# facebookarchive/Surround360

Hardware: AMD Instinct MI355X
Metric: stereo-equirect frames/sec at 8K, 17-cam rig (higher is better)
Workload: dtype f32

## Files before the change

surround360_amd/csrc/api.hip:

```cpp
#include <algorithm>
#include <cstdio>
#include <cstdlib>
#include <cstring>
#include <fstream>
#include <mutex>
#include <sstream>

#include "../../include/s360.h"
#include "../../include/s360_debug.h"
#include "ctx.hpp"
#include "isp.hpp"
#include "render.hpp"

using namespace s360;

static thread_local std::string g_err;

namespace {
std::mutex g_ctxMu;
std::vector<unsigned long long> g_ctxLive;
unsigned long long g_ctxNext = 0;
}
namespace s360 {
bool context_alive(unsigned long long uid) {
// ... 428 lines not shown
    c->op_d.ensure(B * sizeof(void*));
    h2d(c, c->op_a.p, src, B * ns * 4);
    uchar4* down = c->op_b.as<uchar4>();
    float* gray = c->op_c.as<float>();
    float* alpha = gray + B * nd;
    std::vector<const uchar4*> tab(B);
    if (generic) {
      launch_resize_cubic_u8c4_generic(c->st, c->op_a.as<uchar4>(), sw, sh, ns, down, dw, dh, nd, batch);
      launch_gray_alpha(c->st, down, nd, nd, gray, alpha, nd, batch);
    } else {
      for (size_t b = 0; b < B; ++b) tab[b] = c->op_a.as<uchar4>() + ns * b;
      h2d(c, c->op_d.p, tab.data(), B * sizeof(void*));
      S360_HIP(hipMemsetAsync(down, 0x5a, B * nd * 4, c->st));
      launch_entry_downscale(c->st, nullptr, sw, sh, 0, down_out ? down : nullptr, down + B * nd, dw, dh, nd, batch,
                             c->op_d.as<const uchar4*>(), gray, alpha, nd);
    }
    if (down_out) d2h(c, down_out, down, B * nd * 4);
    d2h(c, gray_out, gray, B * nd * sizeof(float));
    d2h(c, alpha_out, alpha, B * nd * sizeof(float));
    if (tiled) *tiled = resize_cubic_u8c4_tiled_fits(sw, sh, dw, dh) ? 1 : 0;
  });
}

int s360_spherical_warp_map(s360_ctx* c, float* map_out, int dw, int dh, const s360_camera* cam, float l, float r,
                            float t, float b) {
  return guard(c, [&] {
    need(c && map_out && cam && dw > 0 && dh > 0, "bad argument");
    c->op_a.ensure((size_t)dw * dh * sizeof(float2));
    build_spherical_map(c, c->op_a.as<float2>(), dw, dh, *cam, l, r, t, b);
    d2h(c, map_out, c->op_a.p, (size_t)dw * dh * sizeof(float2));
  });
}
int s360_bicubic_remap_to_spherical(s360_ctx* c, uint8_t* dst, int dw, int dh, int dc, const uint8_t* src, int sw,
                                    int sh, int sc, const s360_camera* cam, float l, float r, float t, float b) {
  return guard(c, [&] {
    need(c && dst && src && cam, "null argument");
    need((dc == 3 || dc == 4) && (sc == 3 || sc == 4), "channels must be 3 or 4");
    need(!(sc == 4 && dc == 3), "4-channel source: the reference's remap() re-creates the destination with the source's type (ImageWarper.cpp:173) - pass a 4-channel destination");
    FrameState& F = frame_state(c);
    const size_t sn = (size_t)sw * sh, dn = (size_t)dw * dh;
    c->op_a.ensure(dn * sizeof(float2));
    c->op_b.ensure(sn * 4);
    c->op_c.ensure(sn * sizeof(uchar4));
    c->op_d.ensure(dn * sizeof(uchar4));
    build_spherical_map(c, c->op_a.as<float2>(), dw, dh, *cam, l, r, t, b);
    h2d(c, c->op_b.p, src, sn * sc);
    launch_bgr_to_bgra(c->st, c->op_b.as<uint8_t>(), sc, c->op_c.as<uchar4>(), sn);
    launch_remap_cubic_u8c4(c->st, c->op_c.as<uchar4>(), sw, sh, c->op_a.as<float2>(), c->op_d.as<uchar4>(), dw, dh,
                            F.tab.dev, 0, 0, 1);
    if (dc == 4) {
      d2h(c, dst, c->op_d.p, dn * 4);
    } else {
      c->op_e.ensure(dn * 3);
      launch_pack_bgr(c->st, c->op_d.as<uchar4>(), dw, dh, c->op_e.as<uint8_t>());
      d2h(c, dst, c->op_e.p, dn * 3);
    }
  });
}
int s360_combine_lazy_novel_views(s360_ctx* c, const uint8_t* image_l, const uint8_t* image_r, const float* flow_l_to_r,
                                  const float* flow_r_to_l, uint8_t* chunk_l, uint8_t* chunk_r) {
  return guard(c, [&] {
    need(c && image_l && image_r && flow_l_to_r && flow_r_to_l && chunk_l && chunk_r, "null argument");
    FrameState& F = frame_state(c);
    const s360_geometry& g = c->g;
    const int P = F.P, ow = g.overlap_image_width, camH = g.cam_image_height, stripW = c->P.eqr_width / P;
    const size_t on = (size_t)ow * camH, sn = (size_t)stripW * camH;
    c->op_a.ensure(2 * on * 4);
    c->op_b.ensure(2 * on * sizeof(float2));
    c->op_c.ensure(2 * sn * 4);
    h2d(c, c->op_a.p, image_l, on * 4);
    h2d(c, c->op_a.as<uint8_t>() + on * 4, image_r, on * 4);
    h2d(c, c->op_b.p, flow_l_to_r, on * sizeof(float2));
    h2d(c, c->op_b.as<float2>() + on, flow_r_to_l, on * sizeof(float2));
    NovelViewParams nv;
    nv.overlapW = ow; nv.camH = camH; nv.stripW = stripW; nv.numNovelViews = g.num_novel_views;
    nv.numPairs = 1; nv.numLocal = 1;
    nv.camImageWidthHalf = float(g.cam_image_width) * 0.5f;
    nv.disp = g.verge_at_infinity_slab_displacement;
    launch_novel_view(c->st, c->op_a.as<uchar4>(), c->op_b.as<float2>(), c->op_c.as<uchar4>(), nv, 0, 1, F.tab.dev);
    d2h(c, chunk_l, c->op_c.p, sn * 4);
    d2h(c, chunk_r, c->op_c.as<uint8_t>() + sn * 4, sn * 4);
  });
}
static void morph_views_resident(s360_ctx* c, int w, int h, const double* shifts, int n, uint8_t* out_merged, uint8_t* out_from_l,
                                 uint8_t* out_from_r) {
  FrameState& F = frame_state(c);
  const size_t px = (size_t)w * h, V = n;
  c->op_c.ensure(V * px * 4 * (1 + (out_from_l ? 1 : 0) + (out_from_r ? 1 : 0)));
  c->op_d.ensure(V * sizeof(double));
  h2d(c, c->op_d.p, shifts, V * sizeof(double));
  uchar4* merged = c->op_c.as<uchar4>();
  uchar4* fromL = out_from_l ? merged + V * px : nullptr;
  uchar4* fromR = out_from_r ? merged + V * px * (out_from_l ? 2 : 1) : nullptr;
  const char* e = std::getenv("S360_MORPH_VPB");
  {
    ProfScope ps(c->prof, "morph_views");
    launch_morph_views(c->st, c->op_a.as<uchar4>(), c->op_a.as<uchar4>() + px, c->op_b.as<float2>(), c->op_b.as<float2>() + px, w, h,
                       c->op_d.as<double>(), n, merged, fromL, fromR, F.tab.dev, e ? std::atoi(e) : 0);
  }
  d2h(c, out_merged, merged, V * px * 4);
  if (fromL) d2h(c, out_from_l, fromL, V * px * 4);
  if (fromR) d2h(c, out_from_r, fromR, V * px * 4);
}
int s360_generate_novel_views(s360_ctx* c, const uint8_t* image_l, const uint8_t* image_r, const float* flow_l_to_r,
                              const float* flow_r_to_l, int w, int h, const double* shifts, int n, uint8_t* out_merged,
                              uint8_t* out_from_l, uint8_t* out_from_r) {
  return guard(c, [&] {
    need(c && image_l && image_r && flow_l_to_r && flow_r_to_l && shifts && out_merged, "null argument");
    need(w > 0 && h > 0, "image size must be positive");
    need(n >= 1, "at least one shift is required");
    const size_t px = (size_t)w * h;
    c->op_a.ensure(2 * px * 4);
    c->op_b.ensure(2 * px * sizeof(float2));
    h2d(c, c->op_a.p, image_l, px * 4);
    h2d(c, c->op_a.as<uint8_t>() + px * 4, image_r, px * 4);
    h2d(c, c->op_b.p, flow_l_to_r, px * sizeof(float2));
    h2d(c, c->op_b.as<float2>() + px, flow_r_to_l, px * sizeof(float2));
    morph_views_resident(c, w, h, shifts, n, out_merged, out_from_l, out_from_r);
  });
}
int s360_interpolate_views(s360_ctx* c, const char* alg, const uint8_t* image_l, const uint8_t* image_r, int w, int h,
                           const double* shifts, int n, uint8_t* out_merged, uint8_t* out_from_l, uint8_t* out_from_r,
                           float* out_flow_l_to_r, float* out_flow_r_to_l) {
  return guard(c, [&] {
    need(c && alg && image_l && image_r && shifts && out_merged, "null argument");
    need(w >= 4 && h >= 4, "image too small: the reference's bilinear taps need a 2x2 image after the x0.5 entry downscale (PixFlow.h:457-475)");
    need(n >= 1, "at least one shift is required");
    const PixFlowConsts pc = pixflow_consts_by_name(alg);
    const size_t px = (size_t)w * h;
    c->op_a.ensure(2 * px * 4);
    c->op_b.ensure(2 * px * sizeof(float2));
    h2d(c, c->op_a.p, image_l, px * 4);
    h2d(c, c->op_a.as<uint8_t>() + px * 4, image_r, px * 4);
    for (int d = 0; d < 2; ++d) {
      FlowBatch fb;
      fb.add_images(c->op_a.as<uchar4>(), 2, px);
      fb.add_flow(d, 1 - d, c->op_b.as<float2>() + px * d);
      c->flow->compute(c->st, pc, fb, w, h, d == 0 ? S360_HINT_LEFT : S360_HINT_RIGHT);
    }
    morph_views_resident(c, w, h, shifts, n, out_merged, out_from_l, out_from_r);
    if (out_flow_l_to_r) d2h(c, out_flow_l_to_r, c->op_b.p, px * sizeof(float2));
    if (out_flow_r_to_l) d2h(c, out_flow_r_to_l, c->op_b.as<float2>() + px, px * sizeof(float2));
  });
}
int s360_flatten_layers_deghost_prefer_base(s360_ctx* c, const uint8_t* bottom_layer, const uint8_t* top_layer, int w,
                                            int h, uint8_t* out) {
  return guard(c, [&] {
    need(c && bottom_layer && top_layer && out && w > 0 && h > 0, "bad argument");
    FrameState& F = frame_state(c);
    const size_t n = (size_t)w * h;
    c->op_a.ensure(n * 4); c->op_b.ensure(n * 4); c->op_c.ensure(n * 4);
    h2d(c, c->op_a.p, bottom_layer, n * 4);
    h2d(c, c->op_b.p, top_layer, n * 4);
    launch_flatten(c->st, c->op_a.as<uchar4>(), c->op_b.as<uchar4>(), c->op_c.as<uchar4>(), w, h, 0, F.tab.dev);
    d2h(c, out, c->op_c.p, n * 4);
  });
}
int s360_offset_horizontal_wrap(s360_ctx* c, const uint8_t* src, int w, int h, int channels, float offset,
                                uint8_t* out) {
  return guard(c, [&] {
    need(c && src && out && w > 0 && h > 0, "bad argument");
    need(channels == 3 || channels == 4, "channels must be 3 or 4");
    const size_t n = (size_t)w * h;
    c->op_a.ensure(n * 4); c->op_b.ensure(n * 4);
    if (channels == 4) {
      h2d(c, c->op_a.p, src, n * 4);
    } else {
      c->op_c.ensure(n * 3);
      h2d(c, c->op_c.p, src, n * 3);
      launch_bgr_to_bgra(c->st, c->op_c.as<uint8_t>(), 3, c->op_a.as<uchar4>(), n);
    }
    launch_assemble_pano(c->st, c->op_a.as<uchar4>(), 1, h, w, offset, c->op_b.as<uchar4>(), w, h);
    if (channels == 4) {
      d2h(c, out, c->op_b.p, n * 4);
    } else {
      launch_pack_bgr(c->st, c->op_b.as<uchar4>(), w, h, c->op_c.as<uint8_t>());
      d2h(c, out, c->op_c.p, n * 3);
    }
  });
}
int s360_feather_alpha_channel(s360_ctx* c, const uint8_t* src, int w, int h, int erode_size, uint8_t* out) {
  return guard(c, [&] {
    need(c && src && out && w > 0 && h > 0, "bad argument");
    need(erode_size >= 1 && erode_size <= 32, "erode_size must be in 1..32");
    need(erode_size % 2 == 1, "erode_size must be odd (it is the GaussianBlur kernel size, CvUtil.cpp:151)");
    const size_t n = (size_t)w * h;
    c->op_a.ensure(n * 4); c->op_b.ensure(n * 4);
    h2d(c, c->op_a.p, src, n * 4);
    if (erode_size == c->P.std_alpha_feather_size) {
      dev_feather_alpha_to_ext(c, c->op_a.as<uchar4>(), w, h, c->op_b.as<uchar4>(), w);
    } else {
      const std::vector<int> taps = feather_gauss_taps(erode_size);
      c->op_e.ensure(taps.size() * sizeof(int));
      h2d(c, c->op_e.p, taps.data(), taps.size() * sizeof(int));
      dev_feather_alpha_to_ext(c, c->op_a.as<uchar4>(), w, h, c->op_b.as<uchar4>(), w, erode_size, c->op_e.as<int>());
    }
    d2h(c, out, c->op_b.p, n * 4);
  });
}
int s360_pole_to_side_flow(s360_ctx* c, const uint8_t* side, const uint8_t* pole, int pole_rows, uint8_t* warped_out,
                           float* flow_out) {
  return guard(c, [&] {
    need(c && side && pole && warped_out && pole_rows > 0, "bad argument");
    need(c->bottom_idx >= 0, "rig has no bottom camera (pole ramp uses its fov, TRSP:461)");
    const int W = c->P.eqr_width, H = c->P.eqr_height;
    need(pole_rows <= H, "pole_rows larger than eqr_height");
    const int extW = int(float(W) * 1.2f);
    const size_t en = (size_t)W * H, pn = (size_t)W * pole_rows, xn = (size_t)extW * pole_rows;
    c->op_a.ensure(en * 4); c->op_b.ensure(pn * 4); c->op_c.ensure(2 * xn * 4); c->op_d.ensure(xn * sizeof(float2));
    c->op_e.ensure(en * 4);
    h2d(c, c->op_a.p, side, en * 4);
    h2d(c, c->op_b.p, pole, pn * 4);
    uchar4* ext = c->op_c.as<uchar4>();
    dev_feather_alpha_to_ext(c, c->op_a.as<uchar4>(), W, pole_rows, ext, extW);
    launch_extend_wrap(c->st, c->op_b.as<uchar4>(), nullptr, W, pole_rows, ext + xn, extW);
    (void)flow_engine(c, 1);
    FlowBatch fb;
    fb.add_images(ext, 2, xn);
    fb.add_flow(0, 1, c->op_d.as<float2>());
    c->flow_pole->compute(c->st, pixflow_consts_by_name(c->P.polar_flow_alg), fb, extW, pole_rows, S360_HINT_DOWN);
    dev_pole_unit_post(c, ext + xn, c->op_d.as<float2>(), W, pole_rows, extW, c->op_e.as<uchar4>(), H);
    d2h(c, warped_out, c->op_e.p, en * 4);
    if (flow_out) d2h(c, flow_out, c->op_d.p, xn * sizeof(float2));
  });
}
int s360_sharpen(s360_ctx* c, uint8_t* bgr, int w, int h, float sharpening) {
  return guard(c, [&] {
    need(c && bgr && w > 1 && h > 1, "bad argument");
    const size_t n = (size_t)w * h;
    c->op_a.ensure(n * 3); c->op_b.ensure(n * 4); c->op_c.ensure(n * 4); c->op_d.ensure(sharpen_scratch_bytes(w, h));
    h2d(c, c->op_a.p, bgr, n * 3);
    launch_bgr_to_bgra(c->st, c->op_a.as<uint8_t>(), 3, c->op_b.as<uchar4>(), n);
    launch_sharpen(c->st, c->op_b.as<uchar4>(), c->op_c.as<uchar4>(), c->op_d.as<float>(), w, h, 1.0f + sharpening);
    launch_pack_bgr(c->st, c->op_b.as<uchar4>(), w, h, c->op_a.as<uint8_t>());
    d2h(c, bgr, c->op_a.p, n * 3);
  });
}

int s360_frame_upload_side(s360_ctx* c, int side_idx, const uint8_t* img, int w, int h, int channels) {
  return frame_guard(c, [&] { need(c && img && w > 0 && h > 0, "bad argument"); frame_upload_side(c, side_idx, img, w, h, channels); });
}
int s360_frame_upload_top(s360_ctx* c, const uint8_t* bgr, int w, int h) {
  return frame_guard(c, [&] { need(c && bgr && w > 0 && h > 0, "bad argument"); frame_upload_pole(c, true, bgr, w, h); });
}
int s360_frame_upload_bottom(s360_ctx* c, const uint8_t* bgr, int w, int h) {
  return frame_guard(c, [&] { need(c && bgr && w > 0 && h > 0, "bad argument"); frame_upload_pole(c, false, bgr, w, h); });
}
int s360_frame_upload_raw(s360_ctx* c, s360_isp* isp, int camera, const uint16_t* raw16, int w, int h) {
  return frame_guard(c, [&] { need(c && isp && raw16 && w > 0 && h > 0, "bad argument"); frame_upload_raw(c, isp, camera, raw16, 16, w, h); });
}
int s360_frame_upload_packed(s360_ctx* c, s360_isp* isp, int camera, const uint8_t* frame, int bits, int w, int h) {
  return frame_guard(c, [&] {
    need(c && isp && frame && w > 0 && h > 0, "bad argument");
    need(bits == 8 || bits == 12, "packed frames are 8 or 12 bits per pixel");
    frame_upload_raw(c, isp, camera, frame, bits, w, h);
  });
}
int s360_frame_upload_pole_removal(s360_ctx* c, const uint8_t* bottom2, const uint8_t* mask, const uint8_t* mask2, int w,
                                   int h) {
  return frame_guard(c, [&] {
    need(c && bottom2 && mask && mask2 && w > 0 && h > 0, "bad argument");
    frame_upload_pole_removal(c, bottom2, mask, mask2, w, h);
  });
}
int s360_frame_set_prev_pole_removal(s360_ctx* c, const float* flow, const uint8_t* bottom_image, const uint8_t* bottom_image2,
                                     int w, int h) {
  return frame_guard(c, [&] {
    need(c && flow && bottom_image && bottom_image2 && w > 0 && h > 0, "bad argument");
    FrameState& F = frame_state(c);
    const size_t n = (size_t)w * h;
    const int prv = F.last_pr;
    F.prImgs[prv].ensure(2 * n * sizeof(uchar4));
    F.prFlow[prv].ensure(n * sizeof(float2));
    h2d(c, F.prImgs[prv].as<uchar4>(), bottom_image, n * sizeof(uchar4));
    h2d(c, F.prImgs[prv].as<uchar4>() + n, bottom_image2, n * sizeof(uchar4));
    h2d(c, F.prFlow[prv].p, flow, n * sizeof(float2));
    S360_HIP(hipStreamSynchronize(c->st));
    F.have_prev_pr = true;
    F.prevPrGot = 0;
  });
}
int s360_frame_render_pairs(s360_ctx* c, int p0, int p1, int use_prev) {
  return frame_guard(c, [&] { need(c, "null ctx"); frame_render_pairs(c, p0, p1, use_prev); });
}
int s360_frame_finish(s360_ctx* c, int pole_mask, int use_prev) {
  return frame_guard(c, [&] { need(c, "null ctx"); frame_finish(c, pole_mask, use_prev); });
}
int s360_frame_render(s360_ctx* c, int use_prev) {
  return frame_guard(c, [&] {
    need(c, "null ctx");
    frame_render_pairs(c, 0, (int)c->rig.side.size(), use_prev);
    frame_finish(c, 15, use_prev);
  });
}
int s360_set_frame_slots(s360_ctx* c, int n) {
  return frame_guard(c, [&] { need(c, "null ctx"); set_frame_slots(c, n); });
}
int s360_select_frame_slot(s360_ctx* c, int k) {
  return frame_guard(c, [&] {
    need(c, "null ctx");
    need(k >= 0 && k < (int)std::max<size_t>(c->slots.size(), 1), "frame slot out of range");
    c->slot = k;
  });
}
int s360_frame_render_batch(s360_ctx* c, int use_prev) {
  return frame_guard(c, [&] { need(c, "null ctx"); frame_render_batch(c, use_prev); });
}
// ... 295 lines not shown
    png_fetch(c, lk, plan, c->op_d, c->op_b, nullptr, nullptr, nullptr, out, cap, n_out, false);
  });
}
void* s360_host_alloc(size_t bytes) {
  void* p = nullptr;
  if (bytes == 0 || hipHostMalloc(&p, bytes, hipHostMallocPortable) != hipSuccess) {
    (void)hipGetLastError();
    g_err = "s360_host_alloc: hipHostMalloc failed";
    return nullptr;
  }
  std::lock_guard<std::mutex> lk(g_pinMu);
  g_pinBlocks.emplace_back(static_cast<const char*>(p), bytes);
  return p;
}
void s360_host_free(void* p) {
  if (!p) return;
  {
    std::lock_guard<std::mutex> lk(g_pinMu);
    for (size_t i = 0; i < g_pinBlocks.size(); ++i)
      if (g_pinBlocks[i].first == p) { g_pinBlocks.erase(g_pinBlocks.begin() + i); break; }
  }
  (void)hipHostFree(p);
}
int s360_frame_uploads_complete(s360_ctx* c) {
  if (!c) return S360_ERR_INVALID_ARG;
  return guard_l(c, [&](std::unique_lock<std::recursive_mutex>& lk) {
    if (!c->haveUploaded) return;
    if (!c->evUpHost) S360_HIP(hipEventCreateWithFlags(&c->evUpHost, hipEventDisableTiming | hipEventBlockingSync));
    S360_HIP(hipEventRecord(c->evUpHost, c->stUp));
    const hipEvent_t ev = c->evUpHost;
    lk.unlock();
    const hipError_t rc = hipEventSynchronize(ev);
    lk.lock();
    S360_HIP(rc);
  });
}

int s360_set_cubemap_output(s360_ctx* c, int face_w, int face_h, const char* format) {
  return frame_guard(c, [&] {
    need(c, "null ctx");
    if (face_w == 0 || face_h == 0) { c->cube_fw = c->cube_fh = 0; return; }
    need(format, "bad argument");
    const std::string f(format);
    if (f != "video" && f != "photo")
      throw Error(S360_ERR_INVALID_ARG, "unexpected cubemap format: " + f + ". valid formats are: video,photo");
    need(face_w > 0 && face_h > 0 && face_w <= 16384 && face_h <= 16384, "cubemap face size must be in 1..16384 (0 = off)");
    (void)cube_maps(c, face_w, face_h, f == "video");
    c->cube_fw = face_w; c->cube_fh = face_h; c->cube_video = f == "video";
  });
}
int s360_frame_cubemap_size(s360_ctx* c, int whc[3]) {
  return guard(c, [&] {
    need(c && whc, "bad argument");
    if (c->cube_fw <= 0 || c->cube_fh <= 0) throw Error(S360_ERR_STATE, "the cubemap output is off (s360_set_cubemap_output)");
    whc[0] = c->cube_video ? 3 * c->cube_fw : c->cube_fw;
    whc[1] = c->cube_video ? 4 * c->cube_fh : 12 * c->cube_fh;
    whc[2] = 3;
  });
}
static void ensure_download_stream(s360_ctx* c) {
  if (!c->stDown) S360_HIP(hipStreamCreateWithFlags(&c->stDown, hipStreamNonBlocking));
  if (!c->evDown) S360_HIP(hipEventCreateWithFlags(&c->evDown, hipEventDisableTiming | hipEventBlockingSync));
  if (!c->downErr) {
    S360_HIP(hipHostMalloc((void**)&c->downErr, 4 * sizeof(unsigned), hipHostMallocDefault));
    std::memset(c->downErr, 0, 4 * sizeof(unsigned));
  }
}
static int cube_buffer(s360_ctx* c, FrameState& F, int age) {
  need(F.frames_done > age, "that frame has not been rendered");
  need(age == 0 || ((c->pipeline || c->two_outputs) && F.outBGR[F.out_cur ^ 1].p),
       "age 1 needs two output buffers (s360_set_frame_pipelining or s360_set_output_double_buffer)");
  const int b = age == 0 ? F.out_cur : F.out_cur ^ 1;
  if (F.cubeFrame[b] != F.frames_done - 1 - age || !F.cubeBGR[b].p)
    throw Error(S360_ERR_STATE, "that frame was rendered without s360_set_cubemap_output");
  return b;
}
static int download_cubemap_impl(s360_ctx* c, int slot, int age, uint8_t* out_bgr) {
  if (!c) return S360_ERR_INVALID_ARG;
  return guard_l(c, [&](std::unique_lock<std::recursive_mutex>& lk) {
    need(out_bgr && (age == 0 || age == 1), "bad argument (age is 0 = latest enqueued frame or 1 = the one before)");
    FrameState& F = slot_state(c, slot);
    const int b = cube_buffer(c, F, age);
    ensure_download_stream(c);
    if (!F.downRead[b]) S360_HIP(hipEventCreateWithFlags(&F.downRead[b], hipEventDisableTiming));
    S360_HIP(hipStreamWaitEvent(c->stDown, F.outDone[b], 0));
    S360_HIP(hipMemcpyAsync(out_bgr, F.cubeBGR[b].p, (size_t)F.cubeOutW[b] * F.cubeOutH[b] * 3, hipMemcpyDeviceToHost, c->stDown));
    if (F.outErrDev[b].p) S360_HIP(hipMemcpyAsync(c->downErr, F.outErrDev[b].p, 3 * sizeof(unsigned), hipMemcpyDeviceToHost, c->stDown));
    S360_HIP(hipEventRecord(F.downRead[b], c->stDown));
    S360_HIP(hipEventRecord(c->evDown, c->stDown));
    const hipEvent_t ev = c->evDown;
    const unsigned* errw = F.outErrDev[b].p ? c->downErr : nullptr;
    lk.unlock();
    const hipError_t rc = hipEventSynchronize(ev);
    lk.lock();
    S360_HIP(rc);
    if (errw && (errw[0] | errw[1] | errw[2])) {
      for (FlowEngine* e : {c->flow.get(), c->flow_pole.get(), c->flow_pr.get()})
        if (e) (void)e->take_error(c->st);
      throw Error(S360_ERR_HIP, "banded sweep timed out waiting for a neighbour band (results invalid)");
    }
  });
}
int s360_frame_download_cubemap(s360_ctx* c, int age, uint8_t* out_bgr) { return download_cubemap_impl(c, -1, age, out_bgr); }
int s360_frame_download_cubemap_slot(s360_ctx* c, int slot, int age, uint8_t* out_bgr) {
  if (slot < 0) return S360_ERR_INVALID_ARG;
  return download_cubemap_impl(c, slot, age, out_bgr);
}
size_t s360_frame_cubemap_png_bound(s360_ctx* c) {
  size_t n = 0;
  if (!c) return 0;
  (void)guard(c, [&] {
    if (c->cube_fw > 0 && c->cube_fh > 0)
      n = PngPlan::make(c->cube_video ? 3 * c->cube_fw : c->cube_fw, c->cube_video ? 4 * c->cube_fh : 12 * c->cube_fh).file_bound;
  });
  return n;
}
static int download_cubemap_png_impl(s360_ctx* c, int slot, int age, uint8_t* out, size_t cap, size_t* n_out) {
  if (!c) return S360_ERR_INVALID_ARG;
  return guard_l(c, [&](std::unique_lock<std::recursive_mutex>& lk) {
    need(out && n_out && (age == 0 || age == 1), "bad argument (age is 0 = latest enqueued frame or 1 = the one before)");
    FrameState& F = slot_state(c, slot);
    const int b = cube_buffer(c, F, age);
    if (F.cubePngFrame[b] != F.frames_done - 1 - age || !F.cubePngFile[b].p)
      throw Error(S360_ERR_STATE, "that frame was rendered without s360_set_png_encode");
    if (!F.downRead[b]) S360_HIP(hipEventCreateWithFlags(&F.downRead[b], hipEventDisableTiming));
    png_fetch(c, lk, F.cubePngPlan[b], F.cubePngMeta[b], F.cubePngFile[b], F.outDone[b], F.downRead[b], F.outErrDev[b].p, out, cap, n_out);
  });
}
int s360_frame_download_cubemap_png(s360_ctx* c, int age, uint8_t* out, size_t cap, size_t* n_out) {
  return download_cubemap_png_impl(c, -1, age, out, cap, n_out);
}
int s360_frame_download_cubemap_png_slot(s360_ctx* c, int slot, int age, uint8_t* out, size_t cap, size_t* n_out) {
  if (slot < 0) return S360_ERR_INVALID_ARG;
  return download_cubemap_png_impl(c, slot, age, out, cap, n_out);
}

int s360_frame_cubemap(s360_ctx* c, int face_w, int face_h, const char* format, int whc[3], uint8_t* out_bgr) {
  return frame_guard(c, [&] {
    need(c && format && whc, "bad argument");
    const std::string f(format);
    if (f != "video" && f != "photo")
      throw Error(S360_ERR_INVALID_ARG, "unexpected cubemap format: " + f + ". valid formats are: video,photo");
    need(face_w > 0 && face_h > 0 && face_w <= 16384 && face_h <= 16384, "cubemap face size must be in 1..16384");
    whc[0] = f == "video" ? 3 * face_w : face_w;
    whc[1] = f == "video" ? 4 * face_h : 12 * face_h;
    whc[2] = 3;
    if (!out_bgr) return;
    int ow = 0, oh = 0;
    wait_finish_stream(c);
    frame_cubemap(c, face_w, face_h, f == "video", &ow, &oh);
    d2h(c, out_bgr, frame_state(c).cubeOut.p, (size_t)ow * oh * 3);
  });
}
static const void* frame_u8_source(s360_ctx* c, FrameState& F, const std::string& n, int idx, bool pack_eye, int& w, int& h, int& ch) {
  const s360_geometry& g = c->g;
  const int W = c->P.eqr_width, H = c->P.eqr_height, P = F.P;
  const void* src = nullptr;
  w = 0; h = 0; ch = 4;
  const int nloc = F.side_p1 - F.side_p0;
  if (n == "projection") {
    need(idx >= 0 && idx < P && F.sc->proj.p, "projection not available");
    w = g.cam_image_width; h = g.cam_image_height;
    src = F.sc->proj.as<uchar4>() + (size_t)w * h * idx;
  } else if (n == "overlap_l" || n == "overlap_r") {
    need(idx >= F.side_p0 && idx < F.side_p1 && F.overlaps[F.last_side].p, "overlap not available");
    w = g.overlap_image_width; h = g.cam_image_height;
    const int j = idx - F.side_p0 + (n == "overlap_r" ? nloc : 0);
    src = F.overlaps[F.last_side].as<uchar4>() + (size_t)w * h * j;
  } else if (n == "side_pano_l" || n == "side_pano_r") {
    const int e = n == "side_pano_r";
    need(F.panoDbg[e].p, "enable keep_intermediates before rendering");
    w = W; h = H; src = F.panoDbg[e].p;
  } else if (n == "top_spherical") {
    need(F.sc->topSph.p, "not available"); w = W; h = g.top_rows; src = F.sc->topSph.p;
  } else if (n == "bottom_spherical") {
    need(F.sc->botSph.p, "not available"); w = W; h = g.bottom_rows; src = F.sc->botSph.p;
  } else if (n == "pole_warped") {
    need(idx >= 0 && idx < 4 && F.sc->poleWarped[idx].p, "not available"); w = W; h = H; src = F.sc->poleWarped[idx].p;
  } else if (n == "extended_side" || n == "extended_fisheye") {
    need(idx >= 0 && idx < 4 && F.extImgs[F.last_pole].p, "not available");
    w = F.extW; h = idx < 2 ? F.poleRowsT : F.poleRowsB;
    const int slot = n == "extended_side" ? idx : (idx < 2 ? 4 : 5);
    src = F.extImgs[F.last_pole].as<uchar4>() + F.extStride * slot;
  } else if (n == "bottom_image" || n == "bottom_image2") {
    need(F.prImgs[F.last_pr].p && F.have_prev_pr, "not available (pole removal not run)");
    w = F.poleW; h = F.poleH;
    src = F.prImgs[F.last_pr].as<uchar4>() + (n == "bottom_image2" ? (size_t)w * h : 0);
  } else if (n == "eye_l" || n == "eye_r") {
    const int e = n == "eye_r";
    need(F.pano[e].p, "not available");
    w = W; h = H; ch = 3;
    if (pack_eye) {
      c->op_f.ensure((size_t)w * h * 3);
      wait_finish_stream(c);
      launch_pack_bgr(c->st, F.pano[e].as<uchar4>(), w, h, c->op_f.as<uint8_t>());
      src = c->op_f.p;
    }
  } else {
    throw Error(S360_ERR_INVALID_ARG, "unknown intermediate name: " + n);
  }
  return src;
}
int s360_frame_get_u8(s360_ctx* c, const char* name, int idx, int whc[3], uint8_t* dst) {
  return frame_guard(c, [&] {
    need(c && name && whc, "bad argument");
    int w = 0, h = 0, ch = 4;
    const void* src = frame_u8_source(c, frame_state(c), name, idx, dst != nullptr, w, h, ch);
    whc[0] = w; whc[1] = h; whc[2] = ch;
    if (dst) d2h(c, dst, src, (size_t)w * h * ch);
  });
}
size_t s360_png_bound_c(int w, int h, int channels) {
  size_t n = 0;
  (void)guard(nullptr, [&] { n = PngPlan::make(w, h, channels).file_bound; });
  return n;
}
int s360_encode_png_c(s360_ctx* c, const uint8_t* px, int w, int h, int channels, uint8_t* out, size_t cap, size_t* n_out) {
  if (!c) return S360_ERR_INVALID_ARG;
  return guard_l(c, [&](std::unique_lock<std::recursive_mutex>& lk) {
    need(px && out && n_out && w > 0 && h > 0, "bad argument");
    const PngPlan plan = PngPlan::make(w, h, channels);
    const size_t nb = (size_t)w * h * channels;
    c->op_a.ensure((nb + 3) & ~(size_t)3);
    c->op_b.ensure(plan.file_bound);
    S360_HIP(hipMemcpyAsync(c->op_a.p, px, nb, hipMemcpyHostToDevice, c->st));
    png_encode_enqueue(c->st, c->op_a.as<uint8_t>(), plan, c->op_c, c->op_d, c->op_b.as<uint8_t>());
    S360_HIP(hipStreamSynchronize(c->st));
    png_fetch(c, lk, plan, c->op_d, c->op_b, nullptr, nullptr, nullptr, out, cap, n_out, false);
  }, false);
}
static void png_batch_prepare(s360_ctx* c, s360_ctx::PngBatch& B, const std::vector<PngPlan>& plans) {
  if (!B.events) {
    S360_HIP(hipEventCreateWithFlags(&B.evEnc, hipEventDisableTiming));
    S360_HIP(hipEventCreateWithFlags(&B.evRead, hipEventDisableTiming));
    S360_HIP(hipEventCreateWithFlags(&B.evAfter, hipEventDisableTiming));
    B.events = true;
  }
  if (B.haveEnc && hipEventQuery(B.evEnc) != hipSuccess) {
    (void)hipGetLastError();
    S360_HIP(hipEventSynchronize(B.evEnc));
  }
  B.haveEnc = false;
  B.plan = PngBatchPlan::make(plans);
  auto grow = [](void*& p, size_t& have, size_t want) {
    if (have >= want) return;
    if (p) (void)hipHostFree(p);
    p = nullptr;
    have = 0;
    S360_HIP(hipHostMalloc(&p, want, hipHostMallocDefault));
    have = want;
  };
  grow(B.tabHost, B.tabHostBytes, PngBatchPlan::table_bytes(plans.size(), (size_t)B.plan.nbands));
  grow(B.metaHost, B.metaHostBytes, B.plan.meta_records * sizeof(PngBandMeta));
}
static void png_batch_run(s360_ctx* c, s360_ctx::PngBatch& B, const uint8_t* const* px) {
  if (B.haveRead) S360_HIP(hipStreamWaitEvent(c->st, B.evRead, 0));
  png_batch_enqueue(c->st, px, B.plan, B.table, B.tabHost, B.scratch, B.meta, B.files);
  S360_HIP(hipMemcpyAsync(B.metaHost, B.meta.p, B.plan.meta_records * sizeof(PngBandMeta), hipMemcpyDeviceToHost, c->st));
  S360_HIP(hipEventRecord(B.evEnc, c->st));
  B.haveEnc = true;
  ++B.gen;
}
static void png_batch_fetch(s360_ctx* c, std::unique_lock<std::recursive_mutex>& lk, s360_ctx::PngBatch& B, int i, uint8_t* out, size_t cap,
                            size_t* n_out, bool release) {
  if (!B.haveEnc) throw Error(S360_ERR_STATE, "no PNG batch has been encoded");
  need(i >= 0 && (size_t)i < B.plan.img.size(), "PNG index out of range");
  need(out && n_out, "bad argument");
  const PngPlan plan = B.plan.img[(size_t)i];
  const uint8_t* file = B.files.as<uint8_t>() + B.plan.file_off[(size_t)i];
  const PngBandMeta* mh = static_cast<const PngBandMeta*>(B.metaHost) + B.plan.meta0[(size_t)i];
  const unsigned long long gen = B.gen;
  const char* too_small = "png: output buffer too small (s360_frame_state_png_bound / s360_png_bound_c give the size to allocate)";
  if (!c->stDown) S360_HIP(hipStreamCreateWithFlags(&c->stDown, hipStreamNonBlocking));
  std::vector<PngBandMeta> m((size_t)plan.nbands + 1);
  const bool known = hipEventQuery(B.evEnc) == hipSuccess;
  if (!known) (void)hipGetLastError();
  size_t nbytes = std::min(cap, plan.file_bound);
  if (known) {
    std::memcpy(m.data(), mh, m.size() * sizeof(PngBandMeta));
    nbytes = (size_t)m[(size_t)plan.nbands].file_off;
    if (nbytes > plan.file_bound || nbytes + 28 > cap) throw Error(S360_ERR_INVALID_ARG, too_small);
  }
  hipEvent_t ev = nullptr;
  S360_HIP(hipEventCreateWithFlags(&ev, hipEventDisableTiming | hipEventBlockingSync));
  struct Drop { hipEvent_t e; ~Drop() { (void)hipEventDestroy(e); } } drop{ev};
  S360_HIP(hipStreamWaitEvent(c->stDown, B.evEnc, 0));
  S360_HIP(hipMemcpyAsync(out, file, nbytes, hipMemcpyDeviceToHost, c->stDown));
  S360_HIP(hipEventRecord(B.evRead, c->stDown));
  B.haveRead = true;
  S360_HIP(hipEventRecord(ev, c->stDown));
  if (release) lk.unlock();
  const hipError_t rc = hipEventSynchronize(ev);
  if (release) lk.lock();
  S360_HIP(rc);
  if (B.gen != gen) throw Error(S360_ERR_STATE, "the PNG batch was replaced by a later encode while this file was being fetched");
  if (!known) {
    std::memcpy(m.data(), mh, m.size() * sizeof(PngBandMeta));
    const size_t end = (size_t)m[(size_t)plan.nbands].file_off;
    if (end > plan.file_bound || end + 28 > cap) throw Error(S360_ERR_INVALID_ARG, too_small);
  }
  if (release) lk.unlock();
  const size_t n = png_finish_host(out, cap, plan, m.data(), png_crc_threads());
  if (release) lk.lock();
  *n_out = n;
}
int s360_encode_png_batch(s360_ctx* c, int n, const uint8_t* const* px, const int* w, const int* h, const int* channels, uint8_t* const* out,
                          const size_t* cap, size_t* n_out) {
  if (!c) return S360_ERR_INVALID_ARG;
  return guard_l(c, [&](std::unique_lock<std::recursive_mutex>& lk) {
    need(n > 0 && n <= 4096 && px && w && h && channels && out && cap && n_out, "bad argument");
    std::vector<PngPlan> plans;
    std::vector<size_t> at;
    size_t total = 0;
    for (int i = 0; i < n; ++i) {
      need(px[i] && out[i], "bad argument");
      plans.push_back(PngPlan::make(w[i], h[i], channels[i]));
      at.push_back(total);
      total += ((size_t)w[i] * h[i] * channels[i] + 15) & ~(size_t)15;
    }
    c->op_a.ensure(total);
    std::vector<const uint8_t*> dev;
    for (int i = 0; i < n; ++i) {
      dev.push_back(c->op_a.as<uint8_t>() + at[(size_t)i]);
      S360_HIP(hipMemcpyAsync(c->op_a.as<uint8_t>() + at[(size_t)i], px[i], (size_t)w[i] * h[i] * channels[i], hipMemcpyHostToDevice, c->st));
    }
    png_batch_prepare(c, c->opPng, plans);
    png_batch_run(c, c->opPng, dev.data());
    S360_HIP(hipStreamSynchronize(c->st));
    for (int i = 0; i < n; ++i) png_batch_fetch(c, lk, c->opPng, i, out[i], cap[i], &n_out[i], false);
  }, false);
}
int s360_frame_encode_state_pngs(s360_ctx* c, int n, const char* const* names, const int* idx) {
  return frame_guard(c, [&] {
    need(c && n > 0 && n <= 4096 && names && idx, "bad argument");
    FrameState& F = frame_state(c);
    std::vector<PngPlan> plans;
    std::vector<const uint8_t*> px;
    for (int i = 0; i < n; ++i) {
      need(names[i] != nullptr, "bad argument");
      int w = 0, h = 0, ch = 0;
      const void* src = frame_u8_source(c, F, names[i], idx[i], false, w, h, ch);
      need(ch == 4 && src, "only the 4-channel intermediates are encoded as state images");
      plans.push_back(PngPlan::make(w, h, 4));
      px.push_back(static_cast<const uint8_t*>(src));
    }
    s360_ctx::PngBatch& B = c->statePng;
    png_batch_prepare(c, B, plans);
    if (c->st2) {
      S360_HIP(hipEventRecord(B.evAfter, c->st2));
      S360_HIP(hipStreamWaitEvent(c->st, B.evAfter, 0));
    }
    png_batch_run(c, B, px.data());
  });
}
size_t s360_frame_state_png_bound(s360_ctx* c, int i) {
  size_t n = 0;
  if (!c) return 0;
  (void)guard(c, [&] {
    const s360_ctx::PngBatch& B = c->statePng;
    if (!B.haveEnc) throw Error(S360_ERR_STATE, "no PNG batch has been encoded");
    need(i >= 0 && (size_t)i < B.plan.img.size(), "PNG index out of range");
    n = B.plan.img[(size_t)i].file_bound;
  });
  return n;
}
int s360_frame_download_state_png(s360_ctx* c, int i, uint8_t* out, size_t cap, size_t* n_out) {
  if (!c) return S360_ERR_INVALID_ARG;
  return guard_l(c, [&](std::unique_lock<std::recursive_mutex>& lk) { png_batch_fetch(c, lk, c->statePng, i, out, cap, n_out, true); });
}
static const char* const kNotDecodable = "not a banded PNG file of this decoder";
int s360_png_decodable(const uint8_t* file, size_t n, int whc[3], int* band_rows) {
  return guard(nullptr, [&] {
    need(whc && band_rows, "bad argument");
    PngBandedInfo I;
    if (!png_parse_banded(file, n, I)) throw Error(S360_ERR_INVALID_ARG, kNotDecodable);
    whc[0] = I.w; whc[1] = I.h; whc[2] = I.channels;
    *band_rows = I.band_rows;
  });
}
[[noreturn]] static void png_fail(s360_ctx* c, int image, int reason, const std::string& msg) {
  c->pngDecFailImage = image;
  c->pngDecFailReason = reason;
  throw Error(S360_ERR_INVALID_ARG, msg);
}
static std::vector<PngBandedInfo> png_parse_all(s360_ctx* c, int n, const uint8_t* const* files, const size_t* bytes) {
  c->pngDecFailImage = -1;
  c->pngDecFailReason = S360_PNG_DECODE_FAILURE_NONE;
  std::vector<PngBandedInfo> info((size_t)n);
  for (int i = 0; i < n; ++i) {
    need(files[i] != nullptr, "bad argument");
    if (!png_parse_banded(files[i], bytes[i], info[(size_t)i]))
      png_fail(c, i, S360_PNG_DECODE_FAILURE_NOT_DECODABLE, "png decode: image " + std::to_string(i) + ": " + kNotDecodable);
  }
  return info;
}
static void png_decode_checked(s360_ctx* c, int n, const uint8_t* const* files, const std::vector<PngBandedInfo>& info, const std::vector<uint8_t*>& dst) {
  try {
    png_decode_run(c->st, c->pngDec, std::vector<const uint8_t*>(files, files + n), info, dst, c->pngDecStats, &c->prof);
  } catch (const PngDecodeError& e) {
    c->pngDecFailImage = e.image;
    c->pngDecFailReason = S360_PNG_DECODE_FAILURE_DAMAGED;
    throw;
  }
}
int s360_png_decode_failure(s360_ctx* c, int* image, int* reason) {
  if (!c) return S360_ERR_INVALID_ARG;
  return guard(c, [&] {
    need(image && reason, "bad argument");
    *image = c->pngDecFailImage;
    *reason = c->pngDecFailReason;
  });
}
int s360_decode_png_batch(s360_ctx* c, int n, const uint8_t* const* files, const size_t* bytes, uint8_t* const* out, const size_t* cap,
                          int* whc_out) {
  if (!c) return S360_ERR_INVALID_ARG;
  return guard_l(c, [&](std::unique_lock<std::recursive_mutex>&) {
    need(n > 0 && n <= 4096 && files && bytes && out && cap, "bad argument");
    const std::vector<PngBandedInfo> info = png_parse_all(c, n, files, bytes);
    std::vector<size_t> at;
    size_t total = 0;
    for (int i = 0; i < n; ++i) {
      const PngBandedInfo& I = info[(size_t)i];
      const size_t nb = (size_t)I.w * I.h * I.channels;
      need(out[i] != nullptr, "bad argument");
      if (cap[i] < nb) png_fail(c, i, S360_PNG_DECODE_FAILURE_MISMATCH, "png decode: image " + std::to_string(i) + ": output buffer too small");
      at.push_back(total);
      total += (nb + 15) & ~(size_t)15;
    }
    c->op_a.ensure(total);
    std::vector<uint8_t*> dst;
    for (int i = 0; i < n; ++i) dst.push_back(c->op_a.as<uint8_t>() + at[(size_t)i]);
    png_decode_checked(c, n, files, info, dst);
    for (int i = 0; i < n; ++i) {
      const PngBandedInfo& I = info[(size_t)i];
      S360_HIP(hipMemcpyAsync(out[i], dst[(size_t)i], (size_t)I.w * I.h * I.channels, hipMemcpyDeviceToHost, c->st));
      if (whc_out) { whc_out[3 * i] = I.w; whc_out[3 * i + 1] = I.h; whc_out[3 * i + 2] = I.channels; }
    }
    S360_HIP(hipStreamSynchronize(c->st));
  }, false);
}
int s360_png_decode_stats(s360_ctx* c, uint64_t out[4]) {
  if (!c) return S360_ERR_INVALID_ARG;
  return guard(c, [&] {
    need(out != nullptr, "bad argument");
    for (int k = 0; k < 4; ++k) out[k] = c->pngDecStats[k];
  });
}
int s360_png_decode_round_histogram(s360_ctx* c, uint64_t hist[66]) {
  if (!c) return S360_ERR_INVALID_ARG;
  return guard(c, [&] {
    need(hist != nullptr, "bad argument");
    for (int k = 0; k < 66; ++k) hist[k] = c->pngDecStats[4 + k];
  });
}
static void prev_side_arrived(FrameState& F, int pair, unsigned bits) {
  if (F.prevSideGot.size() < (size_t)F.P) F.prevSideGot.resize((size_t)F.P, 0);
  unsigned char& g = F.prevSideGot[(size_t)pair];
  g |= (unsigned char)bits;
  if (g == 15) { g = 0; F.have_prev_side = true; }
}
static void prev_pole_arrived(s360_ctx* c, FrameState& F, int unit, unsigned bits) {
  unsigned char& g = F.prevPoleGot[unit];
  g |= (unsigned char)bits;
  if (g == 7) {
    g = 0;
    F.extW = int(float(c->P.eqr_width) * 1.2f);
    F.extStride = (size_t)F.extW * std::max(c->g.top_rows, c->g.bottom_rows);
    F.poleRowsT = c->g.top_rows;
    F.poleRowsB = c->g.bottom_rows;
    F.have_prev_pole = true;
  }
}
static void prev_pr_arrived(FrameState& F, unsigned bits) {
  F.prevPrGot |= (unsigned char)bits;
  if (F.prevPrGot == 7) { F.prevPrGot = 0; F.have_prev_pr = true; }
}
static void prev_side_block(FrameState& F, int pair, int& j, int& n) {
  need(pair >= 0 && pair < F.P, "pair_idx out of range");
  if (!F.partition_declared) { F.side_p0 = 0; F.side_p1 = F.P; }
  need(pair >= F.side_p0 && pair < F.side_p1, "pair_idx outside the block declared with s360_frame_set_partition");
  j = pair - F.side_p0;
  n = F.side_p1 - F.side_p0;
}
int s360_frame_set_prev_images_png(s360_ctx* c, int n, const char* const* names, const int* idx, const uint8_t* const* files,
                                   const size_t* bytes) {
  return frame_guard(c, [&] {
    need(c && n > 0 && n <= 4096 && names && idx && files && bytes, "bad argument");
    FrameState& F = frame_state(c);
    const std::vector<PngBandedInfo> info = png_parse_all(c, n, files, bytes);
    const size_t on = (size_t)c->g.overlap_image_width * c->g.cam_image_height;
    const int extW = int(float(c->P.eqr_width) * 1.2f);
    const size_t xs = (size_t)extW * std::max(c->g.top_rows, c->g.bottom_rows);
    struct Arrival { int kind, k; unsigned bits; };
    std::vector<uint8_t*> dst;
    std::vector<Arrival> arr;
    int prW = 0, prH = 0;
    for (int i = 0; i < n; ++i) {
      need(names[i] != nullptr, "bad argument");
      const std::string nm(names[i]);
      const PngBandedInfo& I = info[(size_t)i];
      int w = 0, h = 0;
      uchar4* p = nullptr;
      if (nm == "overlap_l" || nm == "overlap_r") {
// ... 252 lines not shown
```

surround360_amd/csrc/render.hip:

```cpp
#include "render.hpp"

#include "isp.hpp"

#include <algorithm>
#include <cmath>
#include <cstdlib>
#include <cstring>

#include "devmath.hpp"

namespace s360 {

std::vector<int> feather_gauss_taps(int erode_size) {
  const int n = erode_size;
  std::vector<int> ik(std::max(n, 1));
  std::vector<float> k(std::max(n, 1));
  const double sigma = erode_size / 2.0f;
  const double sigmaX = sigma > 0 ? sigma : ((n - 1) * 0.5 - 1) * 0.3 + 0.8;
  const double scale2X = -0.5 / (sigmaX * sigmaX);
  double sum = 0;
  for (int i = 0; i < n; ++i) {
    const double x = i - (n - 1) * 0.5;
    k[i] = (float)std::exp(scale2X * x * x);
    sum += k[i];
// ... 441 lines not shown
  s360_ctx::PackedMap& pk = *cache.e.back();
  pk.packed.ensure((size_t)batch * dw * dh * sizeof(unsigned));
  pk.tiles.ensure((size_t)batch * remap_packed_tiles(dw, dh) * 16);
  launch_remap_pack_map(st, map, sw, sh, dw, dh, pk.packed.as<unsigned>(), pk.tiles.p, batch);
  S360_HIP(hipEventCreateWithFlags(&pk.ready, hipEventDisableTiming));
  S360_HIP(hipEventRecord(pk.ready, st));
  pk.sw = sw;
  pk.sh = sh;
  return pk;
}

static void side_stage(s360_ctx* c, const std::vector<int>& slotIds, int p0, int p1, int use_prev) {
  const s360_geometry& g = c->g;
  const int P = (int)c->rig.side.size();
  if (p0 < 0 || p1 > P || p1 < p0) throw Error(S360_ERR_INVALID_ARG, "bad pair range");
  if (c->P.eqr_width % P != 0)
    throw Error(S360_ERR_INVALID_ARG, "eqr_width must be evenly divisible by the number of cameras");
  if (g.num_novel_views != c->P.eqr_width / P)
    throw Error(S360_ERR_INVALID_ARG, "numNovelViews != eqr_width / numCams for this rig");
  Profiler& prof = c->prof;
  hipStream_t st = c->st;
  const int camW = g.cam_image_width, camH = g.cam_image_height, ow = g.overlap_image_width;
  const int stripW = c->P.eqr_width / P;
  const size_t pn = (size_t)camW * camH, on = (size_t)ow * camH;
  const int n = p1 - p0;
  std::vector<FrameState*> Fs;
  for (int k : slotIds) {
    SlotScope ss(c, k);
    FrameState& F = frame_state(c);
    if (!F.have_side) throw Error(S360_ERR_STATE, "side images not uploaded");
    for (int p = p0; p < p1; ++p)
      if (!((F.side_uploaded >> p) & 1) || !((F.side_uploaded >> ((p + 1) % P)) & 1))
        throw Error(S360_ERR_STATE, "side image of camera " + std::to_string(((F.side_uploaded >> p) & 1) ? (p + 1) % P : p) +
                                        " not uploaded (needed by pair " + std::to_string(p) + ")");
    F.sc->proj.ensure(P * pn * sizeof(uchar4));
    F.strips.ensure((size_t)2 * P * camH * stripW * sizeof(uchar4));
    Fs.push_back(&F);
  }
  ensure_maps(c);
  if (n == 0) {
    if (c->evSideSrcFree) { S360_HIP(hipEventRecord(c->evSideSrcFree, st)); c->haveSideSrcFree = true; }
    if (c->pipeline && c->haveStripsFree) S360_HIP(hipStreamWaitEvent(st, c->evStripsFree, 0));
    if (c->pipeline) S360_HIP(hipEventRecord(c->evSideDone, st));
    return;
  }
  if (2 * n * (int)Fs.size() > kMaxFlows) throw Error(S360_ERR_INVALID_ARG, "too many flows for one batch");
  wait_for_uploads(c, st);
  bool usePrev = use_prev != 0;
  for (FrameState* F : Fs) usePrev = usePrev && F->have_prev_side && F->side_p0 == p0 && F->side_p1 == p1;
  for (FrameState* F : Fs) F->cur_side = usePrev ? F->last_side ^ 1 : F->last_side;
  for (FrameState* Fp : Fs) {
    FrameState& F = *Fp;
    const size_t sn = (size_t)F.srcW * F.srcH;
    {
      ProfScope ps(prof, "project_side");
      std::vector<char> need(P, 0);
      for (int p = p0; p < p1; ++p) need[p] = need[(p + 1) % P] = 1;
      for (int i = 0; i < P;) {
        if (!need[i]) { ++i; continue; }
        int j = i;
        while (j < P && need[j]) ++j;
        s360_ctx::PackedMap& pk = ensure_packed(c, c->sidePk, c->sideMaps.as<float2>(), F.srcW, F.srcH, camW, camH, P, st);
        launch_remap_cubic_u8c4_packed(st, F.sideSrc.as<uchar4>() + sn * i, F.srcW, F.srcH, c->sideMaps.as<float2>() + pn * i,
                                       pk.packed.as<unsigned>() + pn * i,
                                       (const char*)pk.tiles.p + 16 * remap_packed_tiles(camW, camH) * i,
                                       F.sc->proj.as<uchar4>() + pn * i, camW, camH, F.tab.dev, 0, 0, 1, j - i);
        i = j;
      }
    }
    const int cur = F.cur_side;
    F.overlaps[cur].ensure(2 * n * on * sizeof(uchar4));
    F.sideFlows.ensure(2 * n * on * sizeof(float2));
    {
      ProfScope ps(prof, "crop_overlaps");
      launch_crop_overlaps(st, F.sc->proj.as<uchar4>(), camW, camH, P, ow, F.overlaps[cur].as<uchar4>(), p0, p1);
    }
  }
  if (c->evSideSrcFree) {
    S360_HIP(hipEventRecord(c->evSideSrcFree, st));
    c->haveSideSrcFree = true;
  }
  {
    (void)flow_engine(c, 0);
    const PixFlowConsts pc = pixflow_consts_by_name(c->P.side_flow_alg);
    for (FrameState* F : Fs) F->have_prev_side = false;
    auto build = [&](bool ltor, bool rtol) {
      FlowBatch fb;
      for (size_t k = 0; k < Fs.size(); ++k) {
        FrameState& F = *Fs[k];
        const int cur = F.cur_side, prv = cur ^ 1;
        const int base = (int)fb.images.size();
        fb.add_images(F.overlaps[cur].as<uchar4>(), 2 * n, on);
        if (usePrev) fb.add_prev_images(F.overlaps[prv].as<uchar4>(), 2 * n, on);
        float2* out = F.sideFlows.as<float2>();
        const float2* pf = usePrev ? F.sideFlows.as<float2>() : nullptr;
        if (ltor)
          for (int j = 0; j < n; ++j) fb.add_flow(base + j, base + n + j, out + on * j, pf ? pf + on * j : nullptr);
        if (rtol)
          for (int j = 0; j < n; ++j) fb.add_flow(base + n + j, base + j, out + on * (n + j), pf ? pf + on * (n + j) : nullptr);
      }
      return fb;
    };
    if (pc.maxPercentage == 0) {
      c->flow->compute(st, pc, build(true, true), ow, camH, S360_HINT_LEFT);
    } else {
      c->flow->compute(st, pc, build(true, false), ow, camH, S360_HINT_LEFT);
      c->flow->compute(st, pc, build(false, true), ow, camH, S360_HINT_RIGHT);
    }
  }
  for (FrameState* Fp : Fs) {
    FrameState& F = *Fp;
    const int cur = F.cur_side;
    {
      ProfScope ps(prof, "novel_view");
      NovelViewParams nv;
      nv.overlapW = ow; nv.camH = camH; nv.stripW = stripW; nv.numNovelViews = g.num_novel_views;
      nv.numPairs = P; nv.numLocal = n;
      nv.camImageWidthHalf = float(camW) * 0.5f;
      nv.disp = g.verge_at_infinity_slab_displacement;
      if (c->pipeline && c->haveStripsFree) S360_HIP(hipStreamWaitEvent(st, c->evStripsFree, 0));
      launch_novel_view(st, F.overlaps[cur].as<uchar4>(), F.sideFlows.as<float2>(), F.strips.as<uchar4>(), nv, p0,
                        p1, F.tab.dev);
    }
    F.side_p0 = p0;
    F.side_p1 = p1;
    F.have_prev_side = true;
    F.last_side = cur;
    F.prevSideGot.clear();
  }
  if (c->pipeline) S360_HIP(hipEventRecord(c->evSideDone, st));
}
void frame_render_pairs(s360_ctx* c, int p0, int p1, int use_prev) { side_stage(c, {c->slot}, p0, p1, use_prev); }

void dev_feather_alpha_to_ext(s360_ctx* c, const uchar4* pano, int cols, int rows, uchar4* ext, int extW, int erode_size,
                              const int* taps) {
  FrameState& F = frame_state(c);
  hipStream_t st = c->st;
  const size_t n = (size_t)cols * rows;
  F.a8a.ensure(n);
  F.a8b.ensure(n);
  const int e = erode_size >= 0 ? erode_size : c->P.std_alpha_feather_size;
  const int ksize = erode_size >= 0 ? erode_size : F.tab.gauss_ksize;
  const int* gik = erode_size >= 0 ? taps : F.tab.gik.as<int>();
  launch_erode_alpha(st, pano, F.a8b.as<uint8_t>(), cols, rows, e);
  if (ksize > 1) {
    launch_gauss_u8(st, F.a8b.as<uint8_t>(), F.a8a.as<uint8_t>(), cols, rows, gik, ksize / 2);
    launch_extend_wrap(st, pano, F.a8a.as<uint8_t>(), cols, rows, ext, extW);
  } else {
    launch_extend_wrap(st, pano, F.a8b.as<uint8_t>(), cols, rows, ext, extW);
  }
}

void dev_pole_unit_post(s360_ctx* c, const uchar4* extFisheye, const float2* flow, int cols, int rows, int extW,
                        uchar4* warped_out, int eqrH) {
  FrameState& F = frame_state(c);
  PoleWarpParams pw;
  pw.cols = cols; pw.rows = rows; pw.extW = extW;
  pw.maxBlendX = int(float(cols) * (1.2f - 1.0f));
  pw.poleCameraRadius = c->ramp.poleCameraRadius;
  pw.phiRampStart = c->ramp.phiRampStart;
  pw.phiMid = c->ramp.phiMid;
  pw.phiRampEnd = c->ramp.phiRampEnd;
  F.sc->warpedExt.ensure((size_t)extW * rows * sizeof(uchar4));
  F.sc->warpPacked.ensure((size_t)extW * rows * sizeof(unsigned));
  F.sc->warpTiles.ensure(remap_packed_tiles(extW, rows) * 16);
  launch_pole_warp_packed(c->st, extFisheye, flow, F.sc->warpedExt.as<uchar4>(), pw, F.tab.dev, F.sc->warpPacked.as<unsigned>(),
                          F.sc->warpTiles.p);
  launch_pole_finish(c->st, F.sc->warpedExt.as<uchar4>(), warped_out, eqrH, pw);
}

namespace {
struct FinishStream {
  s360_ctx* c;
  hipStream_t saved, savedProf;
  explicit FinishStream(s360_ctx* c_) : c(c_), saved(c_->st), savedProf(c_->prof.st) {
    if (c->pipeline) {
      c->st = c->st2;
      c->prof.st = c->st2;
      S360_HIP(hipStreamWaitEvent(c->st2, c->evSideDone, 0));
    }
  }
  ~FinishStream() {
    c->st = saved;
    c->prof.st = savedProf;
  }
};
}

static void finish_stage(s360_ctx* c, const std::vector<int>& slotIds, int pole_mask, int use_prev, int phases = 3,
                         int composite_mask = -1) {
  if (composite_mask < 0) composite_mask = pole_mask;
  if (!(phases & 1)) pole_mask = 0;
  const s360_geometry& g = c->g;
  Profiler& prof = c->prof;
  FinishStream finishStream(c);
  hipStream_t st = c->st;
  const int P = (int)c->rig.side.size(), W = c->P.eqr_width, H = c->P.eqr_height, camH = g.cam_image_height, stripW = W / P;
  const size_t en = (size_t)W * H;
  if (!c->P.enable_top) { pole_mask &= ~3; composite_mask &= ~3; }
  if (!c->P.enable_bottom) { pole_mask &= ~12; composite_mask &= ~12; }
  const int rowsT = g.top_rows, rowsB = g.bottom_rows;
  const int extW = int(float(W) * 1.2f);
  const size_t xs = (size_t)extW * std::max(rowsT, rowsB);
  auto rowsOf = [&](int u) { return u < 2 ? rowsT : rowsB; };
  if (pole_mask) ensure_maps(c);
  bool usePrev = use_prev != 0 && pole_mask != 0;
  for (int k : slotIds) {
    SlotScope ss(c, k);
    FrameState& F = frame_state(c);
    usePrev = usePrev && F.have_prev_pole && F.extW == extW && F.poleRowsT == rowsT && F.poleRowsB == rowsB;
  }
  for (int k : slotIds) {
    SlotScope ss(c, k);
    FrameState& F = frame_state(c);
    F.cur_pole = usePrev ? F.last_pole ^ 1 : F.last_pole;
  }
  for (int k : slotIds) {
    SlotScope ss(c, k);
    FrameState& F = frame_state(c);
    if (!(phases & 1)) {
      if (!F.pano[0].p || !F.pano[1].p) throw Error(S360_ERR_STATE, "composite without assembled panoramas (s360_frame_pole_units first)");
      continue;
    }
    if (!F.strips.p) throw Error(S360_ERR_STATE, "no strips rendered for this frame");
    for (int e = 0; e < 2; ++e) F.pano[e].ensure(en * sizeof(uchar4));
    F.sc->panoTmp.ensure(en * sizeof(uchar4));
    {
      ProfScope ps(prof, "assemble_pano");
      const float sh = g.zero_parallax_novel_view_shift_pixels;
      launch_assemble_pano(st, F.strips.as<uchar4>(), P, camH, stripW, sh, F.pano[0].as<uchar4>(), W, H);
      launch_assemble_pano(st, F.strips.as<uchar4>() + (size_t)P * camH * stripW, P, camH, stripW, -sh,
                           F.pano[1].as<uchar4>(), W, H);
    }
    if (F.keep_intermediates)
      for (int e = 0; e < 2; ++e) {
        F.panoDbg[e].ensure(en * sizeof(uchar4));
        S360_HIP(hipMemcpyAsync(F.panoDbg[e].p, F.pano[e].p, en * sizeof(uchar4), hipMemcpyDeviceToDevice, st));
      }
    if (!pole_mask) continue;
    const int cur = F.cur_pole;
    F.extImgs[cur].ensure(6 * xs * sizeof(uchar4));
    F.poleFlows.ensure(4 * xs * sizeof(float2));
    uchar4* ext = F.extImgs[cur].as<uchar4>();
    wait_for_uploads(c, st);
    {
      ProfScope ps(prof, "project_pole");
      if (pole_mask & 3) {
        if (!F.have_top) throw Error(S360_ERR_STATE, "top image not uploaded");
        F.sc->topSph.ensure((size_t)W * rowsT * sizeof(uchar4));
        const int yfs = rowsT - 1 - c->P.std_alpha_feather_size;
        s360_ctx::PackedMap& pk = ensure_packed(c, c->topPk, c->topMap.as<float2>(), F.topW, F.topH, W, rowsT, 1, st);
        launch_remap_cubic_u8c4_packed(st, F.topSrc.as<uchar4>(), F.topW, F.topH, c->topMap.as<float2>(),
                                       pk.packed.as<unsigned>(), pk.tiles.p, F.sc->topSph.as<uchar4>(), W, rowsT,
                                       F.tab.dev, 1, yfs, c->P.std_alpha_feather_size);
        launch_extend_wrap(st, F.sc->topSph.as<uchar4>(), nullptr, W, rowsT, ext + 4 * xs, extW);
      }
      if (pole_mask & 12) {
        if (!F.have_bottom) throw Error(S360_ERR_STATE, "bottom image not uploaded");
        F.sc->botSph.ensure((size_t)W * rowsB * sizeof(uchar4));
        const int yfs = rowsB - 1 - c->P.std_alpha_feather_size;
        if (c->P.enable_pole_removal) {
          dev_pole_removal(c, F, use_prev != 0);
          s360_ctx::PackedMap& pk = ensure_packed(c, c->botPk, c->botMap.as<float2>(), F.poleW, F.poleH, W, rowsB, 1, st);
          launch_remap_cubic_u8c4_packed(st, F.prMerged.as<uchar4>(), F.poleW, F.poleH, c->botMap.as<float2>(),
                                         pk.packed.as<unsigned>(), pk.tiles.p, F.sc->botSph.as<uchar4>(), W, rowsB,
                                         F.tab.dev, 2, yfs, c->P.std_alpha_feather_size);
        } else {
          s360_ctx::PackedMap& pk = ensure_packed(c, c->botPk, c->botMap.as<float2>(), F.poleW, F.poleH, W, rowsB, 1, st);
          launch_remap_cubic_u8c4_packed(st, F.botSrc.as<uchar4>(), F.poleW, F.poleH, c->botMap.as<float2>(),
                                         pk.packed.as<unsigned>(), pk.tiles.p, F.sc->botSph.as<uchar4>(), W, rowsB,
                                         F.tab.dev, 1, yfs, c->P.std_alpha_feather_size);
        }
        launch_extend_wrap(st, F.sc->botSph.as<uchar4>(), nullptr, W, rowsB, ext + 5 * xs, extW);
      }
    }
    {
      ProfScope ps(prof, "pole_prepare");
      if (pole_mask & 12) {
        for (int e = 0; e < 2; ++e) {
          F.sc->panoFlip[e].ensure(en * sizeof(uchar4));
          launch_flip_both(st, F.pano[e].as<uchar4>(), F.sc->panoFlip[e].as<uchar4>(), W, H, rowsB);
        }
      }
      for (int u = 0; u < 4; ++u)
        if (pole_mask & (1 << u)) {
          const uchar4* side = (u < 2) ? F.pano[u & 1].as<uchar4>() : F.sc->panoFlip[u & 1].as<uchar4>();
          dev_feather_alpha_to_ext(c, side, W, rowsOf(u), ext + u * xs, extW);
        }
    }
  }
  if (c->pipeline && (phases & 1)) {
    S360_HIP(hipEventRecord(c->evStripsFree, st));
    c->haveStripsFree = true;
  }
  if (pole_mask) {
    if (c->evPoleSrcFree) {
      S360_HIP(hipEventRecord(c->evPoleSrcFree, st));
      c->havePoleSrcFree = true;
    }
    (void)flow_engine(c, 1);
    const PixFlowConsts pc = pixflow_consts_by_name(c->P.polar_flow_alg);
    for (int k : slotIds) {
      SlotScope ss(c, k);
      frame_state(c).have_prev_pole = false;
    }
    auto run = [&](int mask, int rows) {
      if (!mask) return;
      FlowBatch fb;
      for (int k : slotIds) {
        SlotScope ss(c, k);
        FrameState& F = frame_state(c);
        const int cur = F.cur_pole, prv = cur ^ 1;
        const uchar4* ext = F.extImgs[cur].as<uchar4>();
        const uchar4* pext = usePrev ? F.extImgs[prv].as<uchar4>() : nullptr;
        int fishIdx[2] = {-1, -1};
        for (int u = 0; u < 4; ++u) {
          if (!(mask & (1 << u))) continue;
          const int pole = u >> 1;
          if (fishIdx[pole] < 0) {
            fishIdx[pole] = (int)fb.images.size();
            fb.images.push_back(ext + (4 + pole) * xs);
            if (usePrev) fb.prev_images.push_back(pext + (4 + pole) * xs);
          }
          const int sideIdx = (int)fb.images.size();
          fb.images.push_back(ext + u * xs);
          if (usePrev) fb.prev_images.push_back(pext + u * xs);
          fb.add_flow(sideIdx, fishIdx[pole], F.poleFlows.as<float2>() + u * xs,
                      usePrev ? F.poleFlows.as<float2>() + u * xs : nullptr);
        }
      }
      c->flow_pole->compute(st, pc, fb, extW, rows, S360_HINT_DOWN);
    };
    if (rowsT == rowsB) {
      run(pole_mask, rowsT);
    } else {
      run(pole_mask & 3, rowsT);
      run(pole_mask & 12, rowsB);
    }
  }
  for (int k : slotIds) {
    SlotScope ss(c, k);
    FrameState& F = frame_state(c);
    if (pole_mask) {
      const int cur = F.cur_pole;
      const uchar4* ext = F.extImgs[cur].as<uchar4>();
      {
        ProfScope ps(prof, "pole_warp");
        for (int u = 0; u < 4; ++u)
          if (pole_mask & (1 << u)) {
            F.sc->poleWarped[u].ensure(en * sizeof(uchar4));
            dev_pole_unit_post(c, ext + (u < 2 ? 4 : 5) * xs, F.poleFlows.as<float2>() + u * xs, W, rowsOf(u), extW,
                               F.sc->poleWarped[u].as<uchar4>(), H);
            F.poleFrame[u] = F.frames_done;
            F.sc->poleOwner[u] = &F;
          }
      }
      F.extW = extW;
      F.extStride = xs;
      F.poleRowsT = rowsT;
      F.poleRowsB = rowsB;
      F.have_prev_pole = true;
      F.last_pole = cur;
      for (unsigned char& got : F.prevPoleGot) got = 0;
    }
    if (!(phases & 2)) continue;
    {
      ProfScope ps(prof, "flatten");
      F.sc->panoTmp.ensure(en * sizeof(uchar4));
      for (int u = 0; u < 4; ++u)
        if ((composite_mask & (1 << u)) && (!F.sc->poleWarped[u].p || F.poleFrame[u] != F.frames_done || F.sc->poleOwner[u] != &F))
          throw Error(S360_ERR_STATE, "composite: the warped layer of pole unit " + std::to_string(u) + " of this frame is neither computed nor received");
      for (int e = 0; e < 2; ++e) {
        if (composite_mask & (1 << e)) {
          launch_flatten(st, F.pano[e].as<uchar4>(), F.sc->poleWarped[e].as<uchar4>(), F.sc->panoTmp.as<uchar4>(), W, H, 0,
                         F.tab.dev);
          std::swap(F.pano[e].p, F.sc->panoTmp.p);
          std::swap(F.pano[e].cap, F.sc->panoTmp.cap);
        }
        if (composite_mask & (4 << e)) {
          launch_flatten(st, F.pano[e].as<uchar4>(), F.sc->poleWarped[2 + e].as<uchar4>(), F.sc->panoTmp.as<uchar4>(), W, H, 1,
                         F.tab.dev);
          std::swap(F.pano[e].p, F.sc->panoTmp.p);
          std::swap(F.pano[e].cap, F.sc->panoTmp.cap);
        }
      }
    }
  }
  if (!(phases & 2)) return;
  if (c->P.sharpening > 0.0) {
    ProfScope ps(prof, "finish");
    std::vector<uchar4*> imgs;
    for (int k : slotIds) {
      SlotScope ss(c, k);
      FrameState& F = frame_state(c);
      for (int e = 0; e < 2; ++e) imgs.push_back(F.pano[e].as<uchar4>());
    }
    SlotScratch& S = *c->slotScratch;
    const int per = std::min(sharpen_max_images(), (int)SlotScratch::kSharpenGroup);
    uchar4* lps[SlotScratch::kSharpenGroup];
    float* scr[SlotScratch::kSharpenGroup];
    for (int i = 0; i < per && i < (int)imgs.size(); ++i) {
      S.sharpLp[i].ensure(en * sizeof(uchar4));
      S.sharpBuf[i].ensure(sharpen_scratch_bytes(W, H));
      lps[i] = S.sharpLp[i].as<uchar4>();
      scr[i] = S.sharpBuf[i].as<float>();
    }
    for (size_t i = 0; i < imgs.size(); i += per) {
      const int n = (int)std::min<size_t>(per, imgs.size() - i);
      launch_sharpen_many(st, imgs.data() + i, lps, scr, n, W, H, 1.0f + (float)c->P.sharpening);
    }
  }
  const bool cube = c->cube_fw > 0 && c->cube_fh > 0;
  if (cube) {
    const int fw = c->cube_fw, fh = c->cube_fh, video = c->cube_video;
    const int cw = video ? 3 * fw : fw, ch = video ? 4 * fh : 12 * fh;
    const s360_ctx::CubeMaps& M = cube_maps(c, fw, fh, video);
    std::vector<const uchar4*> eyes;
    std::vector<uint8_t*> outs;
    const DevTables* tab = nullptr;
    for (int k : slotIds) {
      SlotScope ss(c, k);
      FrameState& F = frame_state(c);
      const int ob = (c->pipeline || c->two_outputs) ? F.out_cur ^ 1 : F.out_cur;
      F.cubeBGR[ob].ensure((size_t)cw * ch * 3);
      if (F.downRead[ob]) S360_HIP(hipStreamWaitEvent(st, F.downRead[ob], 0));
      for (int e = 0; e < 2; ++e) eyes.push_back(F.pano[e].as<uchar4>());
      outs.push_back(F.cubeBGR[ob].as<uint8_t>());
      F.cubeOutW[ob] = cw;
      F.cubeOutH[ob] = ch;
      F.cubeFrame[ob] = F.frames_done;
      tab = &F.tab.dev;
    }
    ProfScope ps(prof, "cubemap_stream");
    launch_cubemap_tiles(st, eyes.data(), outs.data(), (int)outs.size(), W, H, M.maps.as<float2>(), M.packed[video].as<unsigned>(),
                         M.tiles[video].p, fw, fh, video, M.lds_pixels, *tab);
  }
  for (int k : slotIds) {
    SlotScope ss(c, k);
    FrameState& F = frame_state(c);
    {
      ProfScope ps(prof, "finish");
      const int outW = g.out_width, outH = g.out_height, eyeH = outH / 2;
      const int ob = (c->pipeline || c->two_outputs) ? F.out_cur ^ 1 : F.out_cur;
      F.outBGR[ob].ensure((size_t)outW * outH * 3);
      if (!F.outDone[ob]) S360_HIP(hipEventCreateWithFlags(&F.outDone[ob], hipEventDisableTiming));
      if (F.downRead[ob]) S360_HIP(hipStreamWaitEvent(st, F.downRead[ob], 0));
      const bool resize = (outW != W) || (eyeH != H);
      for (int e = 0; e < 2; ++e) {
        uchar4* eye = F.pano[e].as<uchar4>();
        uint8_t* half = F.outBGR[ob].as<uint8_t>() + (size_t)e * outW * eyeH * 3;
        if (resize && launch_resize_cubic_u8c4_to_bgr(st, eye, W, H, half, outW, eyeH)) continue;
        if (resize) {
          F.sc->eyeFinal[e].ensure((size_t)outW * eyeH * sizeof(uchar4));
          launch_resize_cubic_u8c4(st, eye, W, H, en, F.sc->eyeFinal[e].as<uchar4>(), outW, eyeH, (size_t)outW * eyeH, 1);
          eye = F.sc->eyeFinal[e].as<uchar4>();
        }
        launch_pack_bgr(st, eye, outW, eyeH, half);
      }
      if (c->png_encode) {
        ProfScope ps(prof, "png_encode");
        F.pngPlan[ob] = PngPlan::make(outW, outH);
        F.pngFile[ob].ensure(F.pngPlan[ob].file_bound);
        png_encode_enqueue(st, F.outBGR[ob].as<uint8_t>(), F.pngPlan[ob], F.sc->pngScratch, F.pngMeta[ob], F.pngFile[ob].as<uint8_t>());
        F.pngFrame[ob] = F.frames_done;
      }
      if (cube && c->png_encode) {
        ProfScope ps(prof, "png_encode");
        F.cubePngPlan[ob] = PngPlan::make(F.cubeOutW[ob], F.cubeOutH[ob]);
        F.cubePngFile[ob].ensure(F.cubePngPlan[ob].file_bound);
        png_encode_enqueue(st, F.cubeBGR[ob].as<uint8_t>(), F.cubePngPlan[ob], F.sc->pngScratch, F.cubePngMeta[ob],
                           F.cubePngFile[ob].as<uint8_t>());
        F.cubePngFrame[ob] = F.frames_done;
      }
      if (!F.outErrDev[ob].p) {
        F.outErrDev[ob].ensure(4 * sizeof(unsigned));
        S360_HIP(hipMemsetAsync(F.outErrDev[ob].p, 0, 4 * sizeof(unsigned), st));
      }
      {
        FlowEngine* eng[3] = {c->flow.get(), c->flow_pole.get(), c->flow_pr.get()};
        for (int i = 0; i < 3; ++i) {
          if (eng[i] && eng[i]->error_word()) {
            S360_HIP(hipMemcpyAsync(F.outErrDev[ob].as<unsigned>() + i, eng[i]->error_word(), sizeof(unsigned), hipMemcpyDeviceToDevice, st));
          }
        }
      }
      S360_HIP(hipEventRecord(F.outDone[ob], st));
      F.out_cur = ob;
      ++F.frames_done;
    }
  }
}
void frame_finish(s360_ctx* c, int pole_mask, int use_prev) { finish_stage(c, {c->slot}, pole_mask, use_prev); }
void frame_pole_units(s360_ctx* c, int pole_mask, int use_prev) { finish_stage(c, {c->slot}, pole_mask, use_prev, 1, 0); }
void frame_composite(s360_ctx* c, int pole_mask) { finish_stage(c, {c->slot}, 0, 0, 2, pole_mask); }

void frame_render_batch(s360_ctx* c, int use_prev) {
  std::vector<int> ids;
  for (int k = 0; k < (int)std::max<size_t>(c->slots.size(), 1); ++k) ids.push_back(k);
  side_stage(c, ids, 0, (int)c->rig.side.size(), use_prev);
  finish_stage(c, ids, 15, use_prev);
}

void frame_render_slots(s360_ctx* c, const int* slots, int n, int use_prev) {

  const int have = (int)std::max<size_t>(c->slots.size(), 1);
  std::vector<int> ids(slots, slots + n);
  for (int k = 0; k < n; ++k)
    if (ids[k] < 0 || ids[k] >= have || (k > 0 && ids[k] <= ids[k - 1]))
      throw Error(S360_ERR_INVALID_ARG, "frame slots must be distinct, ascending and below the number of slots");
  side_stage(c, ids, 0, (int)c->rig.side.size(), use_prev);
  finish_stage(c, ids, 15, use_prev);
}

namespace {
enum CubeFace { CUBE_BACK = 0, CUBE_LEFT, CUBE_TOP, CUBE_BOTTOM, CUBE_FRONT, CUBE_RIGHT };
void cube_index_to_vec3(float x, float y, int face, float out[3]) {
  const float dir[3] = {x, y, 0.5f};
  out[0] = dir[0]; out[1] = dir[1]; out[2] = dir[2];
  switch (face) {
    case CUBE_BACK: out[0] = dir[0]; out[1] = dir[2]; out[2] = -dir[1]; break;
    case CUBE_LEFT: out[0] = -dir[2]; out[1] = dir[0]; out[2] = -dir[1]; break;
    case CUBE_TOP: break;
    case CUBE_BOTTOM: out[0] = dir[0]; out[1] = -dir[1]; out[2] = -dir[2]; break;
    case CUBE_FRONT: out[0] = -dir[0]; out[1] = -dir[2]; out[2] = -dir[1]; break;
    case CUBE_RIGHT: out[0] = dir[2]; out[1] = -dir[0]; out[2] = -dir[1]; break;
  }
}
void cube_map_entry(float x, float y, int face, int srcCols, int srcRows, float fov, float* srcX, float* srcY) {
  float dir[3];
  cube_index_to_vec3(x, y, face, dir);
  const float r = sqrtf(dir[0] * dir[0] + dir[1] * dir[1]);
  float s2 = 0.f;
  for (int i = 0; i < 3; ++i) s2 += dir[i] * dir[i];
  const double nrm = (double)std::sqrt(s2);
// ... 73 lines not shown
```

surround360_amd/csrc/render.hpp:

```cpp
#pragma once
#include <memory>
#include <string>
#include <vector>

#include "core.hpp"
#include "ctx.hpp"
#include "png.hpp"
#include "render_kernels.hpp"

namespace s360 {

struct Tables {
  DevBuf bi, bf, t10, t5, fs, gik, bw1, bres;
  DevTables dev;
  int gauss_ksize = 0;
  void build(hipStream_t st, int std_alpha_feather_size);
};

void build_spherical_map(s360_ctx* c, float2* map, int dw, int dh, const s360_camera& cam, float l, float r, float t,
                         float b);

struct SlotScratch {
  DevBuf proj;
  DevBuf panoFlip[2], panoTmp;
  DevBuf topSph, botSph;
  DevBuf warpedExt, poleWarped[4];
  const void* poleOwner[4] = {nullptr, nullptr, nullptr, nullptr};
  DevBuf warpPacked, warpTiles;
  DevBuf eyeFinal[2];
  DevBuf pngScratch;
  static constexpr int kSharpenGroup = 32;
  DevBuf sharpLp[kSharpenGroup], sharpBuf[kSharpenGroup];
};

struct FrameState {
  Tables tab;
  std::shared_ptr<SlotScratch> sc;
  int P = 0;
  int srcW = 0, srcH = 0;
  int topW = 0, topH = 0, poleW = 0, poleH = 0;
  unsigned long long side_uploaded = 0;
  bool have_side = false, have_top = false, have_bottom = false;
  DevBuf staging, sideSrc, topSrc, botSrc;
  DevBuf overlaps[2];
  DevBuf sideFlows;
  int side_p0 = 0, side_p1 = 0;
  bool partition_declared = false;
  DevBuf strips;
  DevBuf pano[2];
  DevBuf a8a, a8b, gtmp;
  DevBuf extImgs[2], poleFlows;

  DevBuf outBGR[2];
  hipEvent_t outDone[2] = {nullptr, nullptr};
  DevBuf outErrDev[2];
  hipEvent_t downRead[2] = {nullptr, nullptr};
  DevBuf pngFile[2], pngMeta[2];
  PngPlan pngPlan[2];
  long long pngFrame[2] = {-1, -1};
  int out_cur = 0;
  long long frames_done = 0;
  long long poleFrame[4] = {-1, -1, -1, -1};
  ~FrameState() {
    for (auto& e : outDone) if (e) (void)hipEventDestroy(e);
    for (auto& e : downRead) if (e) (void)hipEventDestroy(e);
  }
  int cur_side = 0, cur_pole = 0, last_side = 0, last_pole = 0;
  bool have_prev_side = false, have_prev_pole = false;
  std::vector<unsigned char> prevSideGot;
  unsigned char prevPoleGot[4] = {0, 0, 0, 0}, prevPrGot = 0;
  int prevPrW = 0, prevPrH = 0;
  bool keep_intermediates = false;
  DevBuf panoDbg[2];
  int extW = 0, poleRowsT = 0, poleRowsB = 0;
  size_t extStride = 0;
  DevBuf botSrc2, prRed[2], prImgs[2], prFlow[2], prTmp, prWarp, prMerged;
  bool have_pr_inputs = false, have_prev_pr = false;
  int last_pr = 0;
  DevBuf cubeOut;
  DevBuf cubeBGR[2];
  int cubeOutW[2] = {0, 0}, cubeOutH[2] = {0, 0};
  long long cubeFrame[2] = {-1, -1};
  DevBuf cubePngFile[2], cubePngMeta[2];
  PngPlan cubePngPlan[2];
  long long cubePngFrame[2] = {-1, -1};
};

FrameState& frame_state(s360_ctx* c);
void frame_upload_side(s360_ctx* c, int idx, const uint8_t* img, int w, int h, int ch);
void frame_upload_pole(s360_ctx* c, bool top, const uint8_t* bgr, int w, int h);
void frame_upload_raw(s360_ctx* c, struct s360_isp* isp, int which, const void* raw, int bits, int inW, int inH);
void frame_upload_pole_removal(s360_ctx* c, const uint8_t* bottom2, const uint8_t* mask, const uint8_t* mask2, int w, int h);
void frame_render_pairs(s360_ctx* c, int p0, int p1, int use_prev);
void frame_finish(s360_ctx* c, int pole_mask, int use_prev);
void frame_pole_units(s360_ctx* c, int pole_mask, int use_prev);
void frame_composite(s360_ctx* c, int pole_mask);
void frame_render_batch(s360_ctx* c, int use_prev);
void frame_render_slots(s360_ctx* c, const int* slots, int n, int use_prev);
void set_frame_slots(s360_ctx* c, int n);
void frame_cubemap(s360_ctx* c, int face_w, int face_h, bool video, int* ow, int* oh);
s360_ctx::CubeMaps& cube_maps(s360_ctx* c, int face_w, int face_h, int video);

void comm_unique_id(void* id128);
const char* comm_library_path();
void comm_init_rank(s360_ctx* c, const void* id128, int rank, int nranks);
void comm_init_all(s360_ctx* const* ctxs, int n);
void comm_destroy(s360_ctx* c);
int comm_size(s360_ctx* c);
int comm_rank(s360_ctx* c);
void frame_gather_strips(s360_ctx* c, const int* bounds, int root);
void frame_exchange_strips(s360_ctx* c, const int* bounds, const int* need_mask);
void frame_gather_pole_layers(s360_ctx* c, const int* owner, int root);
void comm_loopback(s360_ctx* c, int src_pair, int dst_pair);

void dev_feather_alpha_to_ext(s360_ctx* c, const uchar4* pano_top_rows, int cols, int rows, uchar4* ext, int extW,
                              int erode_size = -1, const int* taps = nullptr);
std::vector<int> feather_gauss_taps(int erode_size);
void dev_pole_unit_post(s360_ctx* c, const uchar4* extFisheye, const float2* flow, int cols, int rows, int extW,
                        uchar4* warped_out , int eqrH);

bool host_is_pinned(const void* p, size_t bytes);

FlowEngine& flow_engine(s360_ctx* c, int which);
void flow_engines_follow_pipelining(s360_ctx* c);

}
```

surround360_amd/csrc/render_kernels.hip:

```cpp
#include "render_kernels.hpp"

#include <cstdint>
#include <cstdlib>

#include <algorithm>

#include <stdexcept>

#include "devmath.hpp"

namespace s360 {

__global__ __launch_bounds__(256) void k_bgr_to_bgra(const uint8_t* __restrict__ src, int cn, uchar4* __restrict__ dst,
                                                     size_t n) {
  const size_t i = (size_t)blockIdx.x * blockDim.x + threadIdx.x;
  if (i >= n) return;
  const uint8_t* p = src + i * cn;
  dst[i] = make_uchar4(p[0], p[1], p[2], cn == 4 ? p[3] : 255);
}
__global__ __launch_bounds__(256) void k_prepare_side_src(const uint8_t* __restrict__ src, int cn,
                                                          uchar4* __restrict__ dst, int w, int h, int feather) {
  const int x = blockIdx.x * blockDim.x + threadIdx.x, y = blockIdx.y;
  if (x >= w) return;
  const uint8_t* p = src + ((size_t)y * w + x) * cn;
// ... 189 lines not shown
__global__ __launch_bounds__(RT_W* RT_H) void k_remap_cubic_u8c4_tiled(const uchar4* __restrict__ src, int sw, int sh,
                                                                       MapFn mapfn, uchar4* __restrict__ dst, int dw,
                                                                       int dh, const short* __restrict__ tab,
                                                                       int alpha_mode, int yFeatherStart,
                                                                       int featherSize, size_t sbs, size_t dbs) {
  src += sbs * blockIdx.z;
  dst += dbs * blockIdx.z;
  mapfn.advance(dbs * blockIdx.z);
  __shared__ uchar4 s_tile[RT_CAP];
  __shared__ int s_box[4];
  const int x = blockIdx.x * RT_W + threadIdx.x, y = blockIdx.y * RT_H + threadIdx.y;
  const int tid = threadIdx.y * RT_W + threadIdx.x;
  const bool inside = x < dw && y < dh;
  int sx = 0, sy = 0, fxy = 0;
  bool live = false;
  float2 m = make_float2(0.f, 0.f);
  if (inside) {
    m = mapfn(x, y);
    remap_coord(m.x, m.y, &sx, &sy, &fxy);
    live = !(sx >= sw || sx + 4 <= 0 || sy >= sh || sy + 4 <= 0);
  }
  if (tid == 0) { s_box[0] = INT_MAX; s_box[1] = INT_MIN; s_box[2] = INT_MAX; s_box[3] = INT_MIN; }
  const int mnx = wave_min_i(live ? sx : INT_MAX), mxx = wave_max_i(live ? sx : INT_MIN);
  const int mny = wave_min_i(live ? sy : INT_MAX), mxy = wave_max_i(live ? sy : INT_MIN);
  __syncthreads();
  if ((tid & 63) == 0 && mnx <= mxx) {
    atomicMin(&s_box[0], mnx); atomicMax(&s_box[1], mxx);
    atomicMin(&s_box[2], mny); atomicMax(&s_box[3], mxy);
  }
  __syncthreads();
  const int bx0 = s_box[0], by0 = s_box[2];
  const bool any = bx0 <= s_box[1];
  const int bw = any ? s_box[1] + 4 - bx0 : 0, bh = any ? s_box[3] + 4 - by0 : 0;
  uchar4 o = make_uchar4(0, 0, 0, 0);
  if (any && (long long)bw * bh <= RT_CAP) {
    for (int ly = threadIdx.y; ly < bh; ly += RT_H) {
      const int gy = by0 + ly;
      const bool rowIn = gy >= 0 && gy < sh;
      const uchar4* S = src + (size_t)(rowIn ? gy : 0) * sw;
      for (int lx = threadIdx.x; lx < bw; lx += RT_W) {
        const int gx = bx0 + lx;
        s_tile[ly * bw + lx] = (rowIn && gx >= 0 && gx < sw) ? S[gx] : make_uchar4(0, 0, 0, 0);
      }
    }
    __syncthreads();
    if (live) {
      const uint4* w4 = reinterpret_cast<const uint4*>(tab + fxy * 16);
      const uint4 wa = w4[0], wb = w4[1];
      const unsigned wq[8] = {wa.x, wa.y, wa.z, wa.w, wb.x, wb.y, wb.z, wb.w};
      const unsigned* T = reinterpret_cast<const unsigned*>(s_tile) + (sy - by0) * bw + (sx - bx0);
      int acc[4] = {0, 0, 0, 0};
#pragma unroll
      for (int r = 0; r < 4; ++r) {
        const unsigned p0 = T[r * bw], p1 = T[r * bw + 1], p2 = T[r * bw + 2], p3 = T[r * bw + 3];
        const s16x2 w01 = __builtin_bit_cast(s16x2, wq[2 * r]), w23 = __builtin_bit_cast(s16x2, wq[2 * r + 1]);
#pragma unroll
        for (int ch = 0; ch < 4; ++ch) {
          const unsigned sel = 0x0c040c00u + ch * 0x00010001u;
          const s16x2 lo = __builtin_bit_cast(s16x2, __builtin_amdgcn_perm(p1, p0, sel));
          const s16x2 hi = __builtin_bit_cast(s16x2, __builtin_amdgcn_perm(p3, p2, sel));
          acc[ch] = __builtin_amdgcn_sdot2(lo, w01, acc[ch], false);
          acc[ch] = __builtin_amdgcn_sdot2(hi, w23, acc[ch], false);
        }
      }
      o = make_uchar4((unsigned char)sat_u8((acc[0] + (1 << 14)) >> 15), (unsigned char)sat_u8((acc[1] + (1 << 14)) >> 15),
                      (unsigned char)sat_u8((acc[2] + (1 << 14)) >> 15), (unsigned char)sat_u8((acc[3] + (1 << 14)) >> 15));
    }
  } else if (live) {
    o = remap_cubic_u8c4_at(src, sw, sh, m.x, m.y, tab);
  }
  if (!inside) return;
  if (alpha_mode == 1) {
    int a = 255;
    if (y >= yFeatherStart) {
      const float alpha = 1.0f - (float)(y - yFeatherStart) / (float)featherSize;
      a = (int)(unsigned char)(255.0f * alpha);
    }
    o.w = (unsigned char)a;
  } else if (alpha_mode == 2) {
    if (y >= yFeatherStart) {
      const float alpha = 1.0f - (float)(y - yFeatherStart) / (float)featherSize;
      const unsigned char a = (unsigned char)(255.0f * alpha);
      o.w = o.w < a ? o.w : a;
    }
  }
  dst[(size_t)y * dw + x] = o;
}

constexpr int PT_W = 64, PT_H = 16, PT_TY = 4, PT_CAP = 4096;

template <class MapFn>
__global__ __launch_bounds__(PT_W* PT_TY) void k_remap_pack(MapFn mapfn, int sw, int sh, int dw, int dh,
                                                            unsigned* __restrict__ packed, int4* __restrict__ tiles,
                                                            size_t dbs, int tilesPerImage) {
  mapfn.advance(dbs * blockIdx.z);
  packed += dbs * blockIdx.z;
  tiles += (size_t)tilesPerImage * blockIdx.z;
  __shared__ int s_box[4];
  const int tid = threadIdx.y * PT_W + threadIdx.x;
  const int x = blockIdx.x * PT_W + threadIdx.x;
  int sx[4], sy[4], fxy[4];
  bool live[4];
  int mnx = INT_MAX, mxx = INT_MIN, mny = INT_MAX, mxy = INT_MIN;
  float2 raw[4];
#pragma unroll
  for (int k = 0; k < 4; ++k) raw[k] = mapfn.load(min(x, dw - 1), min((int)(blockIdx.y * PT_H + threadIdx.y + PT_TY * k), dh - 1));
#pragma unroll
  for (int k = 0; k < 4; ++k) {
    const int y = blockIdx.y * PT_H + threadIdx.y + PT_TY * k;
    live[k] = false;
    sx[k] = sy[k] = fxy[k] = 0;
    if (x < dw && y < dh) {
      const float2 m = mapfn.apply(x, y, raw[k]);
      remap_coord(m.x, m.y, &sx[k], &sy[k], &fxy[k]);
      live[k] = !(sx[k] >= sw || sx[k] + 4 <= 0 || sy[k] >= sh || sy[k] + 4 <= 0);
      if (live[k]) {
        mnx = min(mnx, sx[k]); mxx = max(mxx, sx[k]);
        mny = min(mny, sy[k]); mxy = max(mxy, sy[k]);
      }
    }
  }
  if (tid == 0) { s_box[0] = INT_MAX; s_box[1] = INT_MIN; s_box[2] = INT_MAX; s_box[3] = INT_MIN; }
  mnx = wave_min_i(mnx); mxx = wave_max_i(mxx);
  mny = wave_min_i(mny); mxy = wave_max_i(mxy);
  __syncthreads();
  if ((tid & 63) == 0 && mnx <= mxx) {
    atomicMin(&s_box[0], mnx); atomicMax(&s_box[1], mxx);
    atomicMin(&s_box[2], mny); atomicMax(&s_box[3], mxy);
  }
  __syncthreads();
  const int bx0 = s_box[0], by0 = s_box[2];
  const bool any = bx0 <= s_box[1];
  int bw = any ? s_box[1] + 4 - bx0 : 0, bh = any ? s_box[3] + 4 - by0 : 0;
  if (any && ((long long)bw * bh > PT_CAP || bw > 2047 || bh > 1023)) bh = -1;
  if (tid == 0) tiles[(size_t)blockIdx.y * gridDim.x + blockIdx.x] = make_int4(bx0, by0, bw, bh);
#pragma unroll
  for (int k = 0; k < 4; ++k) {
    const int y = blockIdx.y * PT_H + threadIdx.y + PT_TY * k;
    if (x < dw && y < dh)
      packed[(size_t)y * dw + x] = (live[k] && bh > 0) ? (0x80000000u | ((unsigned)(sy[k] - by0) << 21) | ((unsigned)(sx[k] - bx0) << 10) | (unsigned)fxy[k]) : 0u;
  }
}

typedef float f2v __attribute__((ext_vector_type(2)));
typedef unsigned short us2v __attribute__((ext_vector_type(2)));
template <class MapFn, int ALPHA, bool WT = false>
__global__ __launch_bounds__(PT_W* PT_TY) void k_remap_cubic_u8c4_packed(const uchar4* __restrict__ src, int sw, int sh,
                                                                         const unsigned* __restrict__ packed,
                                                                         const int4* __restrict__ tiles, MapFn mapfn,
                                                                         uchar4* __restrict__ dst, int dw, int dh,
                                                                         const short* __restrict__ tab,
                                                                         int yFeatherStart, int featherSize, size_t sbs,
                                                                         size_t dbs, int tilesPerImage,
                                                                         const float* __restrict__ w1, const short* __restrict__ wres) {
  __shared__ __attribute__((aligned(16))) float s_w1[WT ? 256 : 4];
  __shared__ short s_res[WT ? 1024 : 2];
  const TileId tile = xcd_tile();
  src += sbs * tile.z;
  dst += dbs * tile.z;
  packed += dbs * tile.z;
  mapfn.advance(dbs * tile.z);
  __shared__ uchar4 s_tile[PT_CAP];
  const int4 box = tiles[(size_t)tilesPerImage * tile.z + (size_t)tile.y * gridDim.x + tile.x];
  const int bx0 = box.x, by0 = box.y, bw = box.z, bh = box.w;
  const int x = tile.x * PT_W + threadIdx.x;
  unsigned pk[4] = {0u, 0u, 0u, 0u};
  if (bh > 0 && x < dw) {
#pragma unroll
    for (int k = 0; k < 4; ++k) {
      const int y = tile.y * PT_H + threadIdx.y + PT_TY * k;
      if (y < dh) pk[k] = packed[(size_t)y * dw + x];
    }
  }
  if (bh > 0) {
    const unsigned* S32 = reinterpret_cast<const unsigned*>(src);
    unsigned* T32 = reinterpret_cast<unsigned*>(s_tile);
    if (WT) {
      const int tid = threadIdx.y * PT_W + threadIdx.x;
      s_w1[tid] = w1[tid];
      reinterpret_cast<uint2*>(s_res)[tid] = reinterpret_cast<const uint2*>(wres)[tid];
    }
    for (int ly0 = threadIdx.y; ly0 < bh; ly0 += 4 * PT_TY)
      for (int lx0 = threadIdx.x; lx0 < bw; lx0 += 2 * PT_W) {
        unsigned v[4][2];
#pragma unroll
        for (int j = 0; j < 4; ++j) {
          const int ly = ly0 + j * PT_TY, gy = by0 + ly;
          const bool rowIn = ly < bh && gy >= 0 && gy < sh;
#pragma unroll
          for (int i = 0; i < 2; ++i) {
            const int lx = lx0 + i * PT_W, gx = bx0 + lx;
            v[j][i] = (rowIn && lx < bw && gx >= 0 && gx < sw) ? S32[(size_t)gy * sw + gx] : 0u;
          }
        }
#pragma unroll
        for (int j = 0; j < 4; ++j) {
          const int ly = ly0 + j * PT_TY;
#pragma unroll
          for (int i = 0; i < 2; ++i) {
            const int lx = lx0 + i * PT_W;
            if (ly < bh && lx < bw) T32[ly * bw + lx] = v[j][i];
          }
        }
      }
    __syncthreads();
  }
#pragma unroll
  for (int k = 0; k < 4; ++k) {
    const int y = tile.y * PT_H + threadIdx.y + PT_TY * k;
    if (x >= dw || y >= dh) continue;
    uchar4 o = make_uchar4(0, 0, 0, 0);
    if (bh > 0) {
      if (pk[k] & 0x80000000u) {
        const int rx = (pk[k] >> 10) & 2047, ry = (pk[k] >> 21) & 1023;
        unsigned wq[8];
        if (WT) {
          const unsigned fxy = pk[k] & 1023u;
          const float4 wy = *reinterpret_cast<const float4*>(&s_w1[(fxy >> 5) * 4]);
          const float4 wx = *reinterpret_cast<const float4*>(&s_w1[128 + (fxy & 31u) * 4]);
          const int rr = s_res[fxy];
          const f2v x01 = {wx.x, wx.y}, x23 = {wx.z, wx.w};
          const float wyr[4] = {wy.x, wy.y, wy.z, wy.w};
          const f2v magic = {12582912.0f, 12582912.0f};
#pragma unroll
          for (int r = 0; r < 4; ++r) {
            f2v a = x01 * wyr[r], b = x23 * wyr[r];
            if (r == 1) a.y = fminf(a.y, 32767.0f);
            a += magic;
            b += magic;
            wq[2 * r] = __builtin_amdgcn_perm(__float_as_uint(a.y), __float_as_uint(a.x), 0x05040100u);
            wq[2 * r + 1] = __builtin_amdgcn_perm(__float_as_uint(b.y), __float_as_uint(b.x), 0x05040100u);
          }
          const unsigned add = ((unsigned)(rr >> 2) & 0xffffu) << (16 * (rr & 1));
          const unsigned a5 = (rr & 2) ? 0u : add, a7 = (rr & 2) ? add : 0u;
          wq[5] = __builtin_bit_cast(unsigned, (us2v)(__builtin_bit_cast(us2v, wq[5]) + __builtin_bit_cast(us2v, a5)));
          wq[7] = __builtin_bit_cast(unsigned, (us2v)(__builtin_bit_cast(us2v, wq[7]) + __builtin_bit_cast(us2v, a7)));
        } else {
          const uint4* w4 = reinterpret_cast<const uint4*>(tab + (pk[k] & 1023u) * 16);
          const uint4 wa = w4[0], wb = w4[1];
          wq[0] = wa.x; wq[1] = wa.y; wq[2] = wa.z; wq[3] = wa.w; wq[4] = wb.x; wq[5] = wb.y; wq[6] = wb.z; wq[7] = wb.w;
        }
        const unsigned* T = reinterpret_cast<const unsigned*>(s_tile) + ry * bw + rx;
        int acc[4] = {1 << 14, 1 << 14, 1 << 14, 1 << 14};
#pragma unroll
        for (int r = 0; r < 4; ++r) {
          const unsigned p0 = T[r * bw], p1 = T[r * bw + 1], p2 = T[r * bw + 2], p3 = T[r * bw + 3];
          const s16x2 w01 = __builtin_bit_cast(s16x2, wq[2 * r]), w23 = __builtin_bit_cast(s16x2, wq[2 * r + 1]);
#pragma unroll
          for (int ch = 0; ch < (ALPHA == 1 ? 3 : 4); ++ch) {
            const unsigned sel = 0x0c040c00u + ch * 0x00010001u;
            const s16x2 lo = __builtin_bit_cast(s16x2, __builtin_amdgcn_perm(p1, p0, sel));
            const s16x2 hi = __builtin_bit_cast(s16x2, __builtin_amdgcn_perm(p3, p2, sel));
            acc[ch] = __builtin_amdgcn_sdot2(lo, w01, acc[ch], false);
            acc[ch] = __builtin_amdgcn_sdot2(hi, w23, acc[ch], false);
          }
        }
        o = make_uchar4((unsigned char)sat_u8(acc[0] >> 15), (unsigned char)sat_u8(acc[1] >> 15), (unsigned char)sat_u8(acc[2] >> 15),
                        ALPHA == 1 ? (unsigned char)0 : (unsigned char)sat_u8(acc[3] >> 15));
      }
    } else if (bh < 0) {
      const float2 m = mapfn(x, y);
      int sx, sy, fxy;
      remap_coord(m.x, m.y, &sx, &sy, &fxy);
      if (!(sx >= sw || sx + 4 <= 0 || sy >= sh || sy + 4 <= 0)) o = remap_cubic_u8c4_at(src, sw, sh, m.x, m.y, tab);
    }
    if (ALPHA == 1) {
      int a = 255;
      if (y >= yFeatherStart) {
        const float alpha = 1.0f - (float)(y - yFeatherStart) / (float)featherSize;
        a = (int)(unsigned char)(255.0f * alpha);
      }
      o.w = (unsigned char)a;
    } else if (ALPHA == 2) {
      if (y >= yFeatherStart) {
        const float alpha = 1.0f - (float)(y - yFeatherStart) / (float)featherSize;
        const unsigned char a = (unsigned char)(255.0f * alpha);
        o.w = o.w < a ? o.w : a;
      }
    }
    dst[(size_t)y * dw + x] = o;
  }
}

__global__ __launch_bounds__(256) void k_red_mask(const uint8_t* __restrict__ bgr, uint8_t* __restrict__ red, size_t n) {
  const size_t i = (size_t)blockIdx.x * blockDim.x + threadIdx.x;
  if (i >= n) return;
  const uint8_t* p = bgr + i * 3;
  red[i] = (p[0] == 0 && p[1] == 0 && p[2] == 255) ? 1 : 0;
}
__global__ __launch_bounds__(256) void k_circle_alpha(const uchar4* __restrict__ src, const uint8_t* __restrict__ red,
                                                      uchar4* __restrict__ dst, int w, int h, float radius) {
  const int x = blockIdx.x * blockDim.x + threadIdx.x, y = blockIdx.y;
  if (x >= w) return;
  const size_t i = (size_t)y * w + x;
  const float dx = (float)x - (float)w / 2.0f;
  const float dy = (float)y - (float)h / 2.0f;
  const float r = sqrtf(dx * dx + dy * dy);
  const float alpha = r < radius ? 1.0f : 0.0f;
  uchar4 p = src[i];
  p.w = (unsigned char)(alpha * 255.0f);
  if (red && red[i]) p.w = 0;
  dst[i] = p;
}
__global__ __launch_bounds__(256) void k_pole_removal_combine(uchar4* __restrict__ bottom, const uchar4* __restrict__ warped2,
                                                              size_t n) {
  const size_t i = (size_t)blockIdx.x * blockDim.x + threadIdx.x;
  if (i >= n) return;
  uchar4 p1 = bottom[i];
  const uchar4 p2 = warped2[i];
  const float alpha = (float)p1.w / 255.0f, alpha2 = (float)p2.w / 255.0f;
  if (alpha < 1.0f && alpha2 > 0.0f) {
    const float a1 = alpha, a2 = 1.0f - alpha;
    p1.x = (unsigned char)(a1 * (float)p1.x + a2 * (float)p2.x);
    p1.y = (unsigned char)(a1 * (float)p1.y + a2 * (float)p2.y);
    p1.z = (unsigned char)(a1 * (float)p1.z + a2 * (float)p2.z);
    p1.w = 255;
    bottom[i] = p1;
  }
}

__global__ __launch_bounds__(256) void k_crop_overlaps_v2(const uint2* __restrict__ proj, int camW2, int camH, int P,
                                                          int overlapW2, uint2* __restrict__ out, int p0, int n) {
  const int x = blockIdx.x * blockDim.x + threadIdx.x, y = blockIdx.y, j = blockIdx.z;
  if (x >= overlapW2) return;
  const int cam = j < n ? p0 + j : (p0 + (j - n) + 1) % P;
  const int x0 = j < n ? camW2 - overlapW2 : 0;
  out[((size_t)j * camH + y) * overlapW2 + x] = proj[((size_t)cam * camH + y) * camW2 + x0 + x];
}
__global__ __launch_bounds__(256) void k_crop_overlaps(const uchar4* __restrict__ proj, int camW, int camH, int P,
                                                       int overlapW, uchar4* __restrict__ out, int p0, int n) {
  const int x = blockIdx.x * blockDim.x + threadIdx.x, y = blockIdx.y, j = blockIdx.z;
  if (x >= overlapW) return;
  const int cam = j < n ? p0 + j : (p0 + (j - n) + 1) % P;
  const int x0 = j < n ? camW - overlapW : 0;
  out[((size_t)j * camH + y) * overlapW + x] = proj[((size_t)cam * camH + y) * camW + x0 + x];
}

__device__ __forceinline__ float2 remap_cubic_f32c2_introw_at(const float2* __restrict__ src, int sw, int sh, float mx,
                                                              float my, const float* __restrict__ tab) {
  int sx, sy, fxy;
  remap_coord(mx, my, &sx, &sy, &fxy);
  const unsigned width1 = sw - 3 > 0 ? sw - 3 : 0, height1 = sh - 3 > 0 ? sh - 3 : 0;
  if ((fxy >> 5) == 0 && (unsigned)sx < width1 && (unsigned)sy < height1) {
    typedef float f4a8_ __attribute__((ext_vector_type(4), aligned(8)));
    const f4a8_* V = reinterpret_cast<const f4a8_*>(src + (size_t)(sy + 1) * sw + sx);
    const f4a8_ ab = V[0], cd = V[1];
    const float4 wr = *reinterpret_cast<const float4*>(tab + fxy * 16 + 4);
    float2 o;
    o.x = ab.x * wr.x + ab.z * wr.y + cd.x * wr.z + cd.z * wr.w;
    o.y = ab.y * wr.x + ab.w * wr.y + cd.y * wr.z + cd.w * wr.w;
    return o;
  }
  return remap_cubic_f32c2_at(src, sw, sh, mx, my, tab);
}

struct LazySample { uchar4 c; float mag; };
__device__ __forceinline__ LazySample lazy_sample(const uchar4* __restrict__ img, const float2* __restrict__ flow,
                                                  int ow, int oh, float xs, float ys, float t,
                                                  const DevTables& T) {
  const float2 f = remap_cubic_f32c2_introw_at(flow, ow, oh, xs, ys, T.bicubic_f);
  const float wx = xs + f.x * t, wy = ys + f.y * t;
  LazySample s;
  s.c = remap_cubic_u8c4_at(img, ow, oh, wx, wy, T.bicubic_i);
  s.c.w = (unsigned char)(int)((1.0f - t) * (float)s.c.w);
  s.mag = sqrtf(f.x * f.x + f.y * f.y);
  return s;
}
__device__ __forceinline__ uchar4 combine_lazy(uchar4 cL, uchar4 cR, float flowMagL, float flowMagR, float fcols,
                                               const DevTables& T) {
  const unsigned char mx = cL.w > cR.w ? cL.w : cR.w;
  const unsigned char outAlpha = ((double)((float)mx / 255.0f) > 0.1) ? 255 : 0;
  if (cL.w == 0 && cR.w == 0) return make_uchar4(0, 0, 0, outAlpha);
  if (cL.w == 0) return make_uchar4(cR.x, cR.y, cR.z, outAlpha);
  if (cR.w == 0) return make_uchar4(cL.x, cL.y, cL.z, outAlpha);
  const float magL = flowMagL / fcols, magR = flowMagR / fcols;
  float blendL = (float)cL.w, blendR = (float)cR.w;
  const float norm = blendL + blendR;
  blendL /= norm;
  blendR /= norm;
  const int sdiff = abs((int)cL.x - (int)cR.x) + abs((int)cL.y - (int)cR.y) + abs((int)cL.z - (int)cR.z);
  const float deghostCoef = T.tanh10[sdiff];
  const double expL = exp((double)(10.0f * blendL) * (1.0 + (double)(20.0f * magL)));
  const double expR = exp((double)(10.0f * blendR) * (1.0 + (double)(20.0f * magR)));
  const double sumExp = expL + expR + 0.00001;
  const float softmaxL = (float)(expL / sumExp);
  const float softmaxR = (float)(expR / sumExp);
  const float wL = lerpf(blendL, softmaxL, deghostCoef), wR = lerpf(blendR, softmaxR, deghostCoef);
  return make_uchar4((unsigned char)trunc_u8((float)cL.x * wL + (float)cR.x * wR),
                     (unsigned char)trunc_u8((float)cL.y * wL + (float)cR.y * wR),
                     (unsigned char)trunc_u8((float)cL.z * wL + (float)cR.z * wR), 255);
}
constexpr int NV_TW = 64, NV_TH = 4;
__global__ __launch_bounds__(NV_TW* NV_TH) void k_novel_view(const uchar4* __restrict__ overlaps,
                                                             const float2* __restrict__ flows, uchar4* __restrict__ strips,
                                                             NovelViewParams nv, int p0, DevTables T) {
  const TileId tile = xcd_tile();
  const int u = tile.x * NV_TW + (threadIdx.x & (NV_TW - 1)), v = tile.y * NV_TH + (threadIdx.x >> 6);
  if (u >= nv.stripW || v >= nv.camH) return;
  const int j = (int)(tile.z >> 1), pair = p0 + j, eye = tile.z & 1;
  const size_t isz = (size_t)nv.overlapW * nv.camH;
  const uchar4* imgL = overlaps + isz * j;
  const uchar4* imgR = overlaps + isz * (nv.numLocal + j);
  const float2* flowLtoR = flows + isz * j;
  const float2* flowRtoL = flows + isz * (nv.numLocal + j);
  uchar4 out = make_uchar4(0, 0, 0, 0);
  if (u < nv.numNovelViews) {
    const float shift = (float)u / (float)nv.numNovelViews;
    const float slabShift = nv.camImageWidthHalf - (float)(nv.numNovelViews - u);
    const float xs = eye == 0 ? slabShift + nv.disp : slabShift - nv.disp;
    const float ys = (float)v;
    const LazySample a = lazy_sample(imgL, flowRtoL, nv.overlapW, nv.camH, xs, ys, shift, T);
    const LazySample b = lazy_sample(imgR, flowLtoR, nv.overlapW, nv.camH, xs, ys, 1.0f - shift, T);
    out = combine_lazy(a.c, b.c, a.mag, b.mag, (float)nv.stripW, T);
  } else {
    const LazySample a = lazy_sample(imgL, flowRtoL, nv.overlapW, nv.camH, 0.f, 0.f, 0.f, T);
    const LazySample b = lazy_sample(imgR, flowLtoR, nv.overlapW, nv.camH, 0.f, 0.f, 1.0f, T);
    out = combine_lazy(a.c, b.c, a.mag, b.mag, (float)nv.stripW, T);
  }
  strips[(((size_t)eye * nv.numPairs + pair) * nv.camH + v) * nv.stripW + u] = out;
}

__device__ __forceinline__ uchar4 combine_novel(uchar4 cL, float blendL, uchar4 cR, float blendR, float flowMagLR,
                                                float flowMagRL, const DevTables& T) {
  if (cL.w == 0 && cR.w == 0) return make_uchar4(0, 0, 0, 0);
  if (cR.w == 0) return make_uchar4(cL.x, cL.y, cL.z, 255);
  if (cL.w == 0) return make_uchar4(cR.x, cR.y, cR.z, 255);
  const int sdiff = abs((int)cL.x - (int)cR.x) + abs((int)cL.y - (int)cR.y) + abs((int)cL.z - (int)cR.z);
  const float deghostCoef = T.tanh10[sdiff];
  const float alphaL = (float)cL.w / 255.0f, alphaR = (float)cR.w / 255.0f;
  const double expL = exp((double)(10.0f * blendL * alphaL) * (1.0 + (double)(100.0f * flowMagRL)));
  const double expR = exp((double)(10.0f * blendR * alphaR) * (1.0 + (double)(100.0f * flowMagLR)));
  const double sumExp = expL + expR + 0.00001;
  const float softmaxL = (float)(expL / sumExp);
// ... 313 lines not shown
    const int ly = t % IH, lx0 = (t / IH) * 4;
    int acc0 = 0, acc1 = 0, acc2 = 0, acc3 = 0;
    for (int j = 0; j < 2 * r + 4; ++j) {
      const int v = s_a[ly][lx0 + j];
      if (j <= 2 * r) acc0 += (int)__umul24((unsigned)s_k[j], (unsigned)v);
      if (j >= 1 && j - 1 <= 2 * r) acc1 += (int)__umul24((unsigned)s_k[j - 1], (unsigned)v);
      if (j >= 2 && j - 2 <= 2 * r) acc2 += (int)__umul24((unsigned)s_k[j - 2], (unsigned)v);
      if (j >= 3) acc3 += (int)__umul24((unsigned)s_k[j - 3], (unsigned)v);
    }
    s_row[ly][lx0] = acc0; s_row[ly][lx0 + 1] = acc1; s_row[ly][lx0 + 2] = acc2; s_row[ly][lx0 + 3] = acc3;
  }
  __syncthreads();
  for (int t = threadIdx.x; t < GU_TW * (GU_TH / 4); t += 256) {
    const int lx = t & (GU_TW - 1), ly0 = (t >> 6) * 4;
    int acc0 = 0, acc1 = 0, acc2 = 0, acc3 = 0;
    for (int j = 0; j < 2 * r + 4; ++j) {
      const int v = s_row[ly0 + j][lx];
      if (j <= 2 * r) acc0 += (int)__umul24((unsigned)s_k[j], (unsigned)v);
      if (j >= 1 && j - 1 <= 2 * r) acc1 += (int)__umul24((unsigned)s_k[j - 1], (unsigned)v);
      if (j >= 2 && j - 2 <= 2 * r) acc2 += (int)__umul24((unsigned)s_k[j - 2], (unsigned)v);
      if (j >= 3) acc3 += (int)__umul24((unsigned)s_k[j - 3], (unsigned)v);
    }
    const int gx = x0 + lx;
    if (gx >= w) continue;
    const int acc[4] = {acc0, acc1, acc2, acc3};
    const bool vec = gx < (w & ~3);
#pragma unroll
    for (int o = 0; o < 4; ++o) {
      const int gy = y0 + ly0 + o;
      if (gy >= h) continue;
      int v;
      if (exact || !vec) v = gauss_u8_round(acc[o], vec);
      else v = gauss_u8_float_column([&](int j) { return s_row[ly0 + o + r + j][lx]; }, [&](int j) { return s_k[r + j]; }, r);
      out[(size_t)gy * w + gx] = (uint8_t)v;
    }
  }
}
template <int R>
__global__ __launch_bounds__(256) void k_gauss_u8_fixed(const uint8_t* __restrict__ a, uint8_t* __restrict__ out, int w,
                                                        int h, const int* __restrict__ ik) {
  constexpr int IW = GU_TW + 2 * R, IH = GU_TH + 2 * R, NT = 2 * R + 1;
  __shared__ int s_a[IH][IW + 1];
  __shared__ int s_row[IH][GU_TW + 1];
  const int tx = threadIdx.x & (GU_TW - 1), ty = threadIdx.x >> 6;
  const int x0 = blockIdx.x * GU_TW, y0 = blockIdx.y * GU_TH;
  int k[NT];
#pragma unroll
  for (int j = 0; j < NT; ++j) k[j] = ik[j];
  int ksum = 0;
#pragma unroll
  for (int j = 0; j < NT; ++j) ksum += k[j];
  const bool exact = ksum <= 256;
  const int ref = a[(size_t)y0 * w + x0];
  bool same = ref == 0 || ksum == 256;
  if ((w & 3) == 0 && (R & 3) == 3) {
    constexpr int GW = (IW + 1 + 3) / 4;
    constexpr int NG = IH * GW, ITG = (NG + 255) / 256;
    unsigned q[ITG];
#pragma unroll
    for (int it = 0; it < ITG; ++it) {
      const int t = threadIdx.x + 256 * it;
      const int ly = min(t, NG - 1) / GW, g = min(t, NG - 1) - ly * GW;
      const uint8_t* row = a + (size_t)reflect101(y0 - R + ly, h) * w;
      const int gx = x0 - R - 1 + 4 * g;
      if (gx >= 0 && gx < w) {
        q[it] = *reinterpret_cast<const unsigned*>(row + gx);
      } else {
        unsigned v4 = 0;
#pragma unroll
        for (int k = 0; k < 4; ++k) v4 |= (unsigned)row[reflect101(gx + k, w)] << (8 * k);
        q[it] = v4;
      }
    }
#pragma unroll
    for (int it = 0; it < ITG; ++it) {
      const int t = threadIdx.x + 256 * it;
      if (t >= NG) continue;
      const int ly = t / GW, g = t - ly * GW;
      const unsigned v4 = q[it];
#pragma unroll
      for (int k = 0; k < 4; ++k) {
        const int lx = 4 * g + k - 1, v = (int)((v4 >> (8 * k)) & 0xffu);
        if (lx >= 0 && lx < IW) {
          same = same && v == ref;
          s_a[ly][lx] = v;
        }
      }
    }
  } else {
    for (int ly = ty; ly < IH; ly += 4) {
      const uint8_t* row = a + (size_t)reflect101(y0 - R + ly, h) * w;
      for (int lx = tx; lx < IW; lx += GU_TW) {
        const int v = row[reflect101(x0 - R + lx, w)];
        same = same && v == ref;
        s_a[ly][lx] = v;
      }
    }
  }
  if (__syncthreads_and(same)) {
    const int ly = threadIdx.x >> 3, gy = y0 + ly, gx0 = x0 + (threadIdx.x & 7) * 8;
    if (gy < h)
      for (int i = 0; i < 8; ++i)
        if (gx0 + i < w) out[(size_t)gy * w + gx0 + i] = (uint8_t)ref;
    return;
  }
  for (int t = threadIdx.x; t < IH * (GU_TW / 4); t += 256) {
    const int g = t / IH, ly = t - g * IH, lx0 = g * 4;
    int acc0 = 0, acc1 = 0, acc2 = 0, acc3 = 0;
#pragma unroll
    for (int j = 0; j < NT + 3; ++j) {
      const int v = s_a[ly][lx0 + j];
      if (j < NT) acc0 += (int)__umul24((unsigned)k[j], (unsigned)v);
      if (j >= 1 && j - 1 < NT) acc1 += (int)__umul24((unsigned)k[j - 1], (unsigned)v);
      if (j >= 2 && j - 2 < NT) acc2 += (int)__umul24((unsigned)k[j - 2], (unsigned)v);
      if (j >= 3) acc3 += (int)__umul24((unsigned)k[j - 3], (unsigned)v);
    }
    s_row[ly][lx0] = acc0; s_row[ly][lx0 + 1] = acc1; s_row[ly][lx0 + 2] = acc2; s_row[ly][lx0 + 3] = acc3;
  }
  __syncthreads();
  for (int t = threadIdx.x; t < GU_TW * (GU_TH / 4); t += 256) {
    const int lx = t & (GU_TW - 1), ly0 = (t >> 6) * 4;
    int acc[4] = {0, 0, 0, 0};
#pragma unroll
    for (int j = 0; j < NT + 3; ++j) {
      const int v = s_row[ly0 + j][lx];
      if (j < NT) acc[0] += (int)__umul24((unsigned)k[j], (unsigned)v);
      if (j >= 1 && j - 1 < NT) acc[1] += (int)__umul24((unsigned)k[j - 1], (unsigned)v);
      if (j >= 2 && j - 2 < NT) acc[2] += (int)__umul24((unsigned)k[j - 2], (unsigned)v);
      if (j >= 3) acc[3] += (int)__umul24((unsigned)k[j - 3], (unsigned)v);
    }
    const int gx = x0 + lx;
    if (gx >= w) continue;
    const bool vec = gx < (w & ~3);
#pragma unroll
    for (int o = 0; o < 4; ++o) {
      const int gy = y0 + ly0 + o;
      if (gy >= h) continue;
      int v;
      if (exact || !vec) v = gauss_u8_round(acc[o], vec);
      else v = gauss_u8_float_column([&](int j) { return s_row[ly0 + o + R + j][lx]; }, [&](int j) { return ik[R + j]; }, R);
      out[(size_t)gy * w + gx] = (uint8_t)v;
    }
  }
}
__global__ __launch_bounds__(256) void k_extend_wrap(const uchar4* __restrict__ img, const uint8_t* __restrict__ alpha,
                                                     int cols, int rows, uchar4* __restrict__ ext, int extW) {
  const int x = blockIdx.x * blockDim.x + threadIdx.x, y = blockIdx.y;
  if (x >= extW) return;
  const int sx = x % cols;
  uchar4 p = img[(size_t)y * cols + sx];
  if (alpha) p.w = alpha[(size_t)y * cols + sx];
  ext[(size_t)y * extW + x] = p;
}

__global__ __launch_bounds__(256) void k_extend_wrap_v4(const uint4* __restrict__ img, const unsigned* __restrict__ alpha,
                                                        int cols4, int rows, uint4* __restrict__ ext, int extW4) {
  const int x = blockIdx.x * blockDim.x + threadIdx.x, y = blockIdx.y;
  if (x >= extW4) return;
  const int sx = x % cols4;
  uint4 p = img[(size_t)y * cols4 + sx];
  if (alpha) {
    const unsigned a = alpha[(size_t)y * cols4 + sx];
    p.x = (p.x & 0xffffffu) | (a << 24);
    p.y = (p.y & 0xffffffu) | ((a >> 8) << 24);
    p.z = (p.z & 0xffffffu) | ((a >> 16) << 24);
    p.w = (p.w & 0xffffffu) | (a & 0xff000000u);
  }
  ext[(size_t)y * extW4 + x] = p;
}
__device__ __forceinline__ uchar4 pole_finish_px(uchar4 o, uchar4 wr, int x, int y, const PoleWarpParams& pw) {
  if (x < pw.maxBlendX) {
    const float alpha = 1.0f - rampf((float)x, (float)pw.maxBlendX * 0.333f, (float)pw.maxBlendX * 0.667f);
    const float srcB = o.x, srcG = o.y, srcR = o.z, srcA = o.w;
    o.x = (unsigned char)trunc_u8((float)wr.x * alpha + srcB * (1.0f - alpha));
    o.y = (unsigned char)trunc_u8((float)wr.y * alpha + srcG * (1.0f - alpha));
    o.z = (unsigned char)trunc_u8((float)wr.z * alpha + srcR * (1.0f - alpha));
    o.w = (unsigned char)trunc_u8(srcA);
  }
  const float phi = pw.poleCameraRadius * (float)(y + 0.5f) / (float)pw.rows;
  const float a2 = 1.0f - rampf(phi, pw.phiMid, pw.phiRampEnd);
  o.w = (unsigned char)trunc_u8((float)o.w * a2);
  return o;
}
__global__ __launch_bounds__(256) void k_pole_finish(const uchar4* __restrict__ warpedExt, uchar4* __restrict__ out,
                                                     int eqrH, PoleWarpParams pw) {
  const int x = blockIdx.x * blockDim.x + threadIdx.x, y = blockIdx.y;
  if (x >= pw.cols) return;
  uchar4 o = make_uchar4(0, 0, 0, 0);
  if (y < pw.rows) {
    o = warpedExt[(size_t)y * pw.extW + x];
    uchar4 wr = o;
    if (x < pw.maxBlendX) wr = warpedExt[(size_t)y * pw.extW + min(x + pw.cols, pw.extW - 1)];
    o = pole_finish_px(o, wr, x, y, pw);
  }
  out[(size_t)y * pw.cols + x] = o;
}
__global__ __launch_bounds__(256) void k_pole_finish_v4(const uint4* __restrict__ warpedExt, uint4* __restrict__ out, int eqrH,
                                                        PoleWarpParams pw) {
  const int x4 = blockIdx.x * blockDim.x + threadIdx.x, y = blockIdx.y, x = 4 * x4;
  if (x >= pw.cols) return;
  uint4 o = make_uint4(0u, 0u, 0u, 0u);
  if (y < pw.rows) {
    const size_t row = (size_t)y * (pw.extW / 4);
    o = warpedExt[row + x4];
    uint4 wr = o;
    if (x < pw.maxBlendX) wr = warpedExt[row + x4 + pw.cols / 4];
    o.x = __builtin_bit_cast(unsigned, pole_finish_px(__builtin_bit_cast(uchar4, o.x), __builtin_bit_cast(uchar4, wr.x), x, y, pw));
    o.y = __builtin_bit_cast(unsigned, pole_finish_px(__builtin_bit_cast(uchar4, o.y), __builtin_bit_cast(uchar4, wr.y), x + 1, y, pw));
    o.z = __builtin_bit_cast(unsigned, pole_finish_px(__builtin_bit_cast(uchar4, o.z), __builtin_bit_cast(uchar4, wr.z), x + 2, y, pw));
    o.w = __builtin_bit_cast(unsigned, pole_finish_px(__builtin_bit_cast(uchar4, o.w), __builtin_bit_cast(uchar4, wr.w), x + 3, y, pw));
  }
  out[(size_t)y * (pw.cols / 4) + x4] = o;
}

__device__ __forceinline__ uchar4 flatten_px(uchar4 b, uchar4 t, const DevTables& T) {
  const int sdiff = abs((int)b.x - (int)t.x) + abs((int)b.y - (int)t.y) + abs((int)b.z - (int)t.z);
  const float deghostCoef = T.tanh5[sdiff];
  const float alphaR = (float)t.w / 255.0f;
  const float alphaL = 1.0f - alphaR;
  const float softmaxL = T.flat_softmaxL[t.w];
  const float softmaxR = 1.0f - softmaxL;
  const float wL = lerpf(alphaL, softmaxL, deghostCoef), wR = lerpf(alphaR, softmaxR, deghostCoef);
  uchar4 o;
  o.x = (unsigned char)trunc_u8((float)b.x * wL + (float)t.x * wR);
  o.y = (unsigned char)trunc_u8((float)b.y * wL + (float)t.y * wR);
  o.z = (unsigned char)trunc_u8((float)b.z * wL + (float)t.z * wR);
  o.w = t.w > b.w ? t.w : b.w;
  return o;
}
__global__ __launch_bounds__(256) void k_flatten(const uchar4* __restrict__ base, const uchar4* __restrict__ top,
                                                 uchar4* __restrict__ out, int w, int h, int flip_top, DevTables T) {
  const int x = blockIdx.x * blockDim.x + threadIdx.x, y = blockIdx.y;
  if (x >= w) return;
  const uchar4 b = base[(size_t)y * w + x];
  const uchar4 t = flip_top ? top[(size_t)(h - 1 - y) * w + (w - 1 - x)] : top[(size_t)y * w + x];
  out[(size_t)y * w + x] = flatten_px(b, t, T);
}
__global__ __launch_bounds__(256) void k_flatten_v4(const uint4* __restrict__ base, const uint4* __restrict__ top,
                                                    uint4* __restrict__ out, int w4, int h, int flip_top, DevTables T) {
  const int x4 = blockIdx.x * blockDim.x + threadIdx.x, y = blockIdx.y;
  if (x4 >= w4) return;
  const uint4 b = base[(size_t)y * w4 + x4];
  uint4 t;
  if (flip_top) {
    const uint4 r = top[(size_t)(h - 1 - y) * w4 + (w4 - 1 - x4)];
    t = make_uint4(r.w, r.z, r.y, r.x);
  } else {
    t = top[(size_t)y * w4 + x4];
  }
  uint4 o;
  o.x = __builtin_bit_cast(unsigned, flatten_px(__builtin_bit_cast(uchar4, b.x), __builtin_bit_cast(uchar4, t.x), T));
  o.y = __builtin_bit_cast(unsigned, flatten_px(__builtin_bit_cast(uchar4, b.y), __builtin_bit_cast(uchar4, t.y), T));
  o.z = __builtin_bit_cast(unsigned, flatten_px(__builtin_bit_cast(uchar4, b.z), __builtin_bit_cast(uchar4, t.z), T));
  o.w = __builtin_bit_cast(unsigned, flatten_px(__builtin_bit_cast(uchar4, b.w), __builtin_bit_cast(uchar4, t.w), T));
  out[(size_t)y * w4 + x4] = o;
}

__device__ __forceinline__ int border_wrap(int p, int len) {
  if (p < 0) p -= ((p - len + 1) / len) * len;
  if (p >= len) p %= len;
  return p;
}
__global__ __launch_bounds__(256) void k_cubemap(const uchar4* __restrict__ eyeL, const uchar4* __restrict__ eyeR, int sw,
                                                 int sh, const float2* __restrict__ maps , int fw, int fh,
                                                 int video, uint8_t* __restrict__ out, int ow, int oh,
                                                 const short* __restrict__ tab) {
  const int x = blockIdx.x * blockDim.x + threadIdx.x, y = blockIdx.y;
  if (x >= ow) return;
  const int eyeH = oh / 2;
  const int eye = y >= eyeH, ye = y - eye * eyeH;
  int face, i, j;
  if (video) {
    const int col = x / fw, row = ye / fh;
    const int order[6] = {1, 0, 2, 3, 4, 5};
    face = order[row * 3 + col];
    i = fw - 1 - (x - col * fw);
    j = ye - row * fh;
  } else {
    face = ye / fh;
    i = x;
    j = ye - face * fh;
  }
  const float2 m = maps[((size_t)face * fh + j) * fw + i];
  int sx, sy, fxy;
  remap_coord(m.x, m.y, &sx, &sy, &fxy);
  const short* w = tab + fxy * 16;
  const uchar4* src = eye ? eyeR : eyeL;
  int xs[4], ys[4];
#pragma unroll
  for (int q = 0; q < 4; ++q) { xs[q] = border_wrap(sx + q, sw); ys[q] = border_wrap(sy + q, sh); }
  int s0 = 0, s1 = 0, s2 = 0;
#pragma unroll
  for (int r = 0; r < 4; ++r) {
    const uchar4* S = src + (size_t)ys[r] * sw;
#pragma unroll
    for (int q = 0; q < 4; ++q) {
      const uchar4 p = S[xs[q]];
      const int ww = w[r * 4 + q];
      s0 += p.x * ww; s1 += p.y * ww; s2 += p.z * ww;
    }
  }
  uint8_t* o = out + ((size_t)y * ow + x) * 3;
  o[0] = (uint8_t)sat_u8((s0 + (1 << 14)) >> 15);
  o[1] = (uint8_t)sat_u8((s1 + (1 << 14)) >> 15);
  o[2] = (uint8_t)sat_u8((s2 + (1 << 14)) >> 15);
}

constexpr int CT_W = 16, CT_H = 16;
struct CubeJobs {
  const uchar4* eye[2 * kCubeMaxSlots];
  uint8_t* out[kCubeMaxSlots];
};
struct CubeGeom { int fw, fh, video, ow, eyeH, txN, tyN; };
__device__ __forceinline__ void cube_face_slot(const CubeGeom& G, int s, int* fx0, int* fy0, int* list) {
  if (G.video) {
    const int row = s >= 3, col = s - 3 * row;
    *fx0 = col * G.fw; *fy0 = row * G.fh; *list = s < 2 ? 1 - s : s;
  } else {
    *fx0 = 0; *fy0 = s * G.fh; *list = s;
  }
}
__device__ __forceinline__ size_t cube_map_index(const CubeGeom& G, int list, int lx, int ly) {
  return ((size_t)list * G.fh + ly) * G.fw + (G.video ? G.fw - 1 - lx : lx);
}

template <int CAP>
__global__ __launch_bounds__(64) void k_cubemap_pack(const float2* __restrict__ maps , int sw, int sh, CubeGeom G,
                                                     unsigned* __restrict__ packed , int4* __restrict__ tiles) {
  int fx0, fy0, list;
  cube_face_slot(G, blockIdx.z, &fx0, &fy0, &list);
  const int lx0 = blockIdx.x * CT_W + (threadIdx.x & 3) * 4, ly = blockIdx.y * CT_H + (threadIdx.x >> 2);
  const int half = sw >> 1;
  int sx[4], sy[4], fxy[4];
  int mnx = INT_MAX, mxx = INT_MIN, mns = INT_MAX, mxs = INT_MIN, mny = INT_MAX, mxy = INT_MIN;
#pragma unroll
  for (int k = 0; k < 4; ++k) {
    sx[k] = sy[k] = fxy[k] = 0;
    if (lx0 + k < G.fw && ly < G.fh) {
      const float2 m = maps[cube_map_index(G, list, lx0 + k, ly)];
      remap_coord(m.x, m.y, &sx[k], &sy[k], &fxy[k]);
      const int xs = sx[k] + (sx[k] < half ? sw : 0);
      mnx = min(mnx, sx[k]); mxx = max(mxx, sx[k]);
      mns = min(mns, xs); mxs = max(mxs, xs);
      mny = min(mny, sy[k]); mxy = max(mxy, sy[k]);
    }
  }
  mnx = wave_min_i(mnx); mxx = wave_max_i(mxx);
  mns = wave_min_i(mns); mxs = wave_max_i(mxs);
  mny = wave_min_i(mny); mxy = wave_max_i(mxy);
  const bool shifted = mxs - mns < mxx - mnx;
  const int bx0 = shifted ? mns : mnx, by0 = mny;
  const int bw = (shifted ? mxs : mxx) + 4 - bx0;
  int bh = mxy + 4 - by0;
  if ((long long)bw * bh > CAP || bw > 2047 || bh > 1023 || bx0 < -sw || bx0 + bw > 3 * sw || by0 < -sh || by0 + bh > 2 * sh) bh = -1;
  if (threadIdx.x == 0) tiles[((size_t)blockIdx.z * G.tyN + blockIdx.y) * G.txN + blockIdx.x] = make_int4(bx0, by0, bw, bh);
#pragma unroll
  for (int k = 0; k < 4; ++k)
    if (lx0 + k < G.fw && ly < G.fh) {
      const int xk = shifted ? sx[k] + (sx[k] < half ? sw : 0) : sx[k];
      packed[(size_t)(fy0 + ly) * G.ow + fx0 + lx0 + k] =
          bh > 0 ? (0x80000000u | ((unsigned)(sy[k] - by0) << 21) | ((unsigned)(xk - bx0) << 10) | (unsigned)fxy[k]) : 0u;
    }
}

__device__ __forceinline__ unsigned cubemap_px_gather(const uchar4* __restrict__ src, int sw, int sh, float2 m,
                                                      const short* __restrict__ tab) {
  int sx, sy, fxy;
  remap_coord(m.x, m.y, &sx, &sy, &fxy);
  const short* w = tab + fxy * 16;
  int xs[4], ys[4];
#pragma unroll
  for (int q = 0; q < 4; ++q) { xs[q] = border_wrap(sx + q, sw); ys[q] = border_wrap(sy + q, sh); }
  int s0 = 1 << 14, s1 = 1 << 14, s2 = 1 << 14;
#pragma unroll
  for (int r = 0; r < 4; ++r) {
    const uchar4* S = src + (size_t)ys[r] * sw;
#pragma unroll
    for (int q = 0; q < 4; ++q) {
      const uchar4 p = S[xs[q]];
      const int ww = w[r * 4 + q];
      s0 += p.x * ww; s1 += p.y * ww; s2 += p.z * ww;
    }
  }
  return (unsigned)sat_u8(s0 >> 15) | ((unsigned)sat_u8(s1 >> 15) << 8) | ((unsigned)sat_u8(s2 >> 15) << 16);
}

template <int CAP>
__global__ __launch_bounds__(64) void k_cubemap_tiles(CubeJobs J, int sw, int sh, const float2* __restrict__ maps,
                                                      const unsigned* __restrict__ packed, const int4* __restrict__ tiles,
                                                      CubeGeom G, const short* __restrict__ tab) {
  __shared__ unsigned s_tile[CAP];
  const TileId tile = xcd_tile();
  const int s = tile.y / G.tyN, ty = tile.y - s * G.tyN;
  const uchar4* __restrict__ src = J.eye[tile.z];
  uint8_t* __restrict__ out = J.out[tile.z >> 1] + (size_t)(tile.z & 1) * G.eyeH * G.ow * 3;
  int fx0, fy0, list;
  cube_face_slot(G, s, &fx0, &fy0, &list);
  const int4 box = tiles[((size_t)s * G.tyN + ty) * G.txN + tile.x];
  const int bx0 = box.x, by0 = box.y, bw = box.z, bh = box.w;
  const int lx0 = tile.x * CT_W + (threadIdx.x & 3) * 4, ly = ty * CT_H + (threadIdx.x >> 2);
  const bool vec = (G.fw & 3) == 0;
// ... 144 lines not shown
#pragma unroll
      for (int kk = 0; kk < IIR_CH; ++kk)
        pre[kk] = reinterpret_cast<const unsigned*>(X)[iir_px<ROWS>(g, min(chain0 + kk, g.nchains - 1), pos)];
    } else {
      const int ch = min(chain0 + cl, g.nchains - 1);
#pragma unroll
      for (int i = 0; i < IIR_CH; ++i) {
        const int e = min(t * IIR_T + 4 * i + rl, g.n - 1);
        pre[i] = reinterpret_cast<const unsigned*>(X)[(size_t)iir_bnd<ROWS>(e + 1, g.n) * g.w + ch];
      }
    }
  };
  auto stage_tile = [&]() {
#pragma unroll
    for (int kk = 0; kk < IIR_CH; ++kk) {
      if (ROWS) s_in[kk * IIR_LD + lane] = pre[kk];
      else s_in[cl * IIR_LD + 4 * kk + rl] = pre[kk];
    }
  };
  const float am = 1.0f - alpha;
  const unsigned char* sb = reinterpret_cast<const unsigned char*>(s_in) + (size_t)k * IIR_LD * 4 + c;
  float v;
  {
    const uchar4 p0 = X[iir_px<ROWS>(g, min(chain0 + k, g.nchains - 1), 0)];
    v = c == 0 ? (float)p0.x : c == 1 ? (float)p0.y : c == 2 ? (float)p0.z : (float)p0.w;
  }
  load_tile(0);
  for (int t = 0; t < ntiles; ++t) {
    ck[(size_t)t * 64] = v;
    stage_tile();
    S360_WAVE_SYNC();
    if (t + 1 < ntiles) load_tile(t + 1);
    const int cnt = min(IIR_T, g.n - t * IIR_T);
    int j = 0;
    for (; j + 8 <= cnt; j += 8) {
      float ip[8];
#pragma unroll
      for (int q = 0; q < 8; ++q) ip[q] = (float)sb[(j + q) * 4] * am;
#pragma unroll
      for (int q = 0; q < 8; ++q) v = ip[q] + v * alpha;
    }
    for (; j < cnt; ++j) v = (float)sb[j * 4] * am + v * alpha;
    S360_WAVE_SYNC();
  }
  const float b_last = v;
  load_tile(ntiles - 1);
  float ck_next = ck[(size_t)(ntiles - 1) * 64];
  for (int t = ntiles - 1; t >= 0; --t) {
    const float b_before = ck_next;
    stage_tile();
    S360_WAVE_SYNC();
    if (t > 0) {
      load_tile(t - 1);
      ck_next = ck[(size_t)(t - 1) * 64];
    }
    unsigned img[IIR_CH];
    if (FUSE) {
#pragma unroll
      for (int kk = 0; kk < IIR_CH; ++kk) {
        const int p = ROWS ? lane : 4 * kk + rl, chn = min(chain0 + (ROWS ? kk : cl), g.nchains - 1), e = min(t * IIR_T + p, g.n - 1);
        img[kk] = reinterpret_cast<const unsigned*>(out)[iir_px<ROWS>(g, chn, e)];
      }
    }
    const int cnt = min(IIR_T, g.n - t * IIR_T);
    float b[IIR_T];
    {
      float u = b_before;
#pragma unroll
      for (int j = 0; j < IIR_T; ++j) {
        u = (float)sb[j * 4] * am + u * alpha;
        b[j] = u;
      }
    }
    const float b_first = t > 0 ? b_before : ROWS ? b_last : b[1];
    unsigned char* so = reinterpret_cast<unsigned char*>(s_out) + (size_t)k * IIR_LD * 4 + c;
#pragma unroll
    for (int j = IIR_T - 1; j >= 0; --j) {
      if (j < cnt) {
        v = (j > 0 ? b[j > 0 ? j - 1 : 0] : b_first) * am + v * alpha;
        so[j * 4] = c == 3 ? (unsigned char)255 : (unsigned char)clamp255(v);
      }
    }
    S360_WAVE_SYNC();
#pragma unroll
    for (int kk = 0; kk < IIR_CH; ++kk) {
      const int p = ROWS ? lane : 4 * kk + rl, chn = chain0 + (ROWS ? kk : cl), e = t * IIR_T + p;
      if (e < g.n) {
        if (chn < g.nchains) {
          const unsigned lw = s_out[(ROWS ? kk : cl) * IIR_LD + p];
          const size_t o = iir_px<ROWS>(g, chn, e);
          if (FUSE) {
            uchar4 px = __builtin_bit_cast(uchar4, img[kk]);
            auto f = [&](unsigned char pc, unsigned lc) -> unsigned char {
              const float lf = (float)lc;
              const float hp = (float)pc - lf;
              const float ng = hp == 0.0f ? 0.0f : 1.0f;
              return (unsigned char)clamp255(lf + hp * ng * amount);
            };
            px.x = f(px.x, lw & 255u); px.y = f(px.y, (lw >> 8) & 255u); px.z = f(px.z, (lw >> 16) & 255u);
            out[o] = px;
          } else {
            reinterpret_cast<unsigned*>(out)[o] = lw;
          }
        }
      }
    }
  }
}

__global__ __launch_bounds__(256) void k_u16_high_byte(const unsigned short* __restrict__ src, uint8_t* __restrict__ dst,
                                                       size_t n) {
  const size_t i = (size_t)blockIdx.x * blockDim.x + threadIdx.x;
  if (i < n) dst[i] = (uint8_t)(src[i] >> 8);
}

static inline unsigned cdiv(size_t a, size_t b) { return (unsigned)((a + b - 1) / b); }

void launch_u16_high_byte(hipStream_t st, const unsigned short* src, uint8_t* dst, size_t n) {
  hipLaunchKernelGGL(k_u16_high_byte, dim3(cdiv(n, 256)), dim3(256), 0, st, src, dst, n);
}

void launch_bgr_to_bgra(hipStream_t st, const uint8_t* src, int channels, uchar4* dst, size_t n) {
  hipLaunchKernelGGL(k_bgr_to_bgra, dim3(cdiv(n, 256)), dim3(256), 0, st, src, channels, dst, n);
}
void launch_prepare_side_src(hipStream_t st, const uint8_t* src, int channels, uchar4* dst, int w, int h, int feather) {
  hipLaunchKernelGGL(k_prepare_side_src, dim3(cdiv(w, 256), h), dim3(256), 0, st, src, channels, dst, w, h, feather);
}
void launch_spherical_map(hipStream_t st, float2* map, int dw, int dh, const DevCamera& cam, const float* cosX,
                          const float* sinX, const float* cosY, const float* sinY) {
  dim3 blk(64, 4);
  hipLaunchKernelGGL(k_spherical_map, dim3(cdiv(dw, 64), cdiv(dh, 4)), blk, 0, st, map, dw, dh, cam, cosX, sinX, cosY,
                     sinY);
}
void launch_remap_cubic_u8c4(hipStream_t st, const uchar4* src, int sw, int sh, const float2* map, uchar4* dst, int dw,
                             int dh, const DevTables& T, int alpha_mode, int yFeatherStart, int featherSize, int batch) {
  MapFromBuffer mf{map, dw};
  hipLaunchKernelGGL((k_remap_cubic_u8c4_tiled<MapFromBuffer>), dim3(cdiv(dw, RT_W), cdiv(dh, RT_H), batch),
                     dim3(RT_W, RT_H), 0, st, src, sw, sh, mf, dst, dw, dh, T.bicubic_i, alpha_mode, yFeatherStart,
                     featherSize, (size_t)sw * sh, (size_t)dw * dh);
}
size_t remap_packed_tiles(int dw, int dh) { return (size_t)cdiv(dw, PT_W) * cdiv(dh, PT_H); }
void launch_remap_pack_map(hipStream_t st, const float2* map, int sw, int sh, int dw, int dh, unsigned* packed, void* tiles,
                           int batch) {
  MapFromBuffer mf{map, dw};
  hipLaunchKernelGGL((k_remap_pack<MapFromBuffer>), dim3(cdiv(dw, PT_W), cdiv(dh, PT_H), batch), dim3(PT_W, PT_TY), 0, st, mf, sw,
                     sh, dw, dh, packed, reinterpret_cast<int4*>(tiles), (size_t)dw * dh, (int)remap_packed_tiles(dw, dh));
}
static bool remap_rebuild_weights() {
  static const bool on = [] { const char* e = std::getenv("S360_REMAP_REBUILD_WEIGHTS"); return !(e && e[0] == '0'); }();
  return on;
}
void launch_remap_cubic_u8c4_packed(hipStream_t st, const uchar4* src, int sw, int sh, const float2* map, const unsigned* packed,
                                    const void* tiles, uchar4* dst, int dw, int dh, const DevTables& T, int alpha_mode,
                                    int yFeatherStart, int featherSize, int batch) {
  MapFromBuffer mf{map, dw};
  const dim3 grid(cdiv(dw, PT_W), cdiv(dh, PT_H), batch), block(PT_W, PT_TY);
  const int4* t4 = reinterpret_cast<const int4*>(tiles);
  const size_t sbs = (size_t)sw * sh, dbs = (size_t)dw * dh;
  const int nt = (int)remap_packed_tiles(dw, dh);
  const bool wt = remap_rebuild_weights() && T.bicubic_res;
#define S360_RP(A, W)                                                                                                              \
  hipLaunchKernelGGL((k_remap_cubic_u8c4_packed<MapFromBuffer, A, W>), grid, block, 0, st, src, sw, sh, packed, t4, mf, dst, dw, dh, \
                     T.bicubic_i, yFeatherStart, featherSize, sbs, dbs, nt, T.bicubic_w1, T.bicubic_res)
  if (alpha_mode == 1) { if (wt) S360_RP(1, true); else S360_RP(1, false); }
  else if (alpha_mode == 2) { if (wt) S360_RP(2, true); else S360_RP(2, false); }
  else { if (wt) S360_RP(0, true); else S360_RP(0, false); }
#undef S360_RP
}
void launch_remap_by_flow(hipStream_t st, const uchar4* src, int w, int h, const float2* flow, uchar4* dst,
                          const DevTables& T) {
  MapFromFlowAdd mf{flow, w};
  hipLaunchKernelGGL((k_remap_cubic_u8c4_tiled<MapFromFlowAdd>), dim3(cdiv(w, RT_W), cdiv(h, RT_H), 1), dim3(RT_W, RT_H), 0, st,
                     src, w, h, mf, dst, w, h, T.bicubic_i, 0, 0, 1, (size_t)0, (size_t)0);
}
void launch_red_mask(hipStream_t st, const uint8_t* bgr, uint8_t* red, size_t n) {
  hipLaunchKernelGGL(k_red_mask, dim3(cdiv(n, 256)), dim3(256), 0, st, bgr, red, n);
}
void launch_circle_alpha(hipStream_t st, const uchar4* src, const uint8_t* red, uchar4* dst, int w, int h, float radius) {
  hipLaunchKernelGGL(k_circle_alpha, dim3(cdiv(w, 256), h), dim3(256), 0, st, src, red, dst, w, h, radius);
}
void launch_pole_removal_combine(hipStream_t st, uchar4* bottom, const uchar4* warped2, size_t n) {
  hipLaunchKernelGGL(k_pole_removal_combine, dim3(cdiv(n, 256)), dim3(256), 0, st, bottom, warped2, n);
}
void launch_crop_overlaps(hipStream_t st, const uchar4* proj, int camW, int camH, int P, int overlapW, uchar4* out,
                          int p0, int p1) {
  const int n = p1 - p0;
  if (n <= 0) return;
  if ((camW & 1) == 0 && (overlapW & 1) == 0 && (reinterpret_cast<uintptr_t>(proj) & 7) == 0 && (reinterpret_cast<uintptr_t>(out) & 7) == 0)
    hipLaunchKernelGGL(k_crop_overlaps_v2, dim3(cdiv(overlapW / 2, 256), camH, 2 * n), dim3(256), 0, st,
                       reinterpret_cast<const uint2*>(proj), camW / 2, camH, P, overlapW / 2, reinterpret_cast<uint2*>(out), p0, n);
  else
    hipLaunchKernelGGL(k_crop_overlaps, dim3(cdiv(overlapW, 256), camH, 2 * n), dim3(256), 0, st, proj, camW, camH, P,
                       overlapW, out, p0, n);
}
void launch_novel_view(hipStream_t st, const uchar4* overlaps, const float2* flows, uchar4* strips,
                       const NovelViewParams& nv, int p0, int p1, const DevTables& T) {
  if (p1 <= p0) return;
  hipLaunchKernelGGL(k_novel_view, dim3(cdiv(nv.stripW, NV_TW), cdiv(nv.camH, NV_TH), 2 * (p1 - p0)), dim3(NV_TW * NV_TH), 0, st,
                     overlaps, flows, strips, nv, p0, T);
}
void launch_morph_views(hipStream_t st, const uchar4* imgL, const uchar4* imgR, const float2* flowLtoR, const float2* flowRtoL,
                        int w, int h, const double* shifts, int n, uchar4* merged, uchar4* fromL, uchar4* fromR,
                        const DevTables& T, int views_per_block) {
  if (n <= 0) return;
  int vpb = views_per_block > 0 ? min(views_per_block, n) : n;
  if (cdiv(n, vpb) > 65535u) vpb = (int)cdiv(n, 65535);
  hipLaunchKernelGGL(k_morph_views, dim3(cdiv(w, NV_TW), cdiv(h, NV_TH), cdiv(n, vpb)), dim3(NV_TW * NV_TH), 0, st, imgL, imgR,
                     flowLtoR, flowRtoL, w, h, shifts, n, vpb, merged, fromL, fromR, T);
}
void launch_assemble_pano(hipStream_t st, const uchar4* strips_eye, int P, int camH, int stripW, float offset,
                          uchar4* pano, int eqrW, int eqrH) {
  const int padAbove = (eqrH - camH) / 2;
  hipLaunchKernelGGL(k_assemble_pano, dim3(cdiv(cdiv(eqrW, 4), 256), eqrH), dim3(256), 0, st, strips_eye, P, camH, stripW, offset,
                     pano, eqrW, eqrH, padAbove);
}
void launch_flip_both(hipStream_t st, const uchar4* src, uchar4* dst, int w, int h, int rows) {
  hipLaunchKernelGGL(k_flip_both, dim3(cdiv(w, 256), rows), dim3(256), 0, st, src, dst, w, h);
}
void launch_erode_alpha(hipStream_t st, const uchar4* img, uint8_t* out, int w, int h, int e) {
  if (e > ER_MAXE) throw std::runtime_error("featherAlphaChannel: erode size above 32 is not supported");
  if (e == 31 && (w & 1) == 0)
    hipLaunchKernelGGL((k_erode_cross_fixed<31>), dim3(cdiv(w, ERF_TW), cdiv(h, ERF_TH)), dim3(256), 0, st, img, out, w, h);
  else
    hipLaunchKernelGGL(k_erode_cross_tiled, dim3(cdiv(w, ER_TW), cdiv(h, ER_TH)), dim3(256), 0, st, img, out, w, h, e);
}
void launch_gauss_u8(hipStream_t st, const uint8_t* a, uint8_t* out, int w, int h, const int* ik, int r) {
  if (r > GU_MAXR) throw std::runtime_error("featherAlphaChannel: Gaussian radius above 16 is not supported");
  if (r == 15)
    hipLaunchKernelGGL((k_gauss_u8_fixed<15>), dim3(cdiv(w, GU_TW), cdiv(h, GU_TH)), dim3(256), 0, st, a, out, w, h, ik);
  else
    hipLaunchKernelGGL(k_gauss_u8_tiled, dim3(cdiv(w, GU_TW), cdiv(h, GU_TH)), dim3(256), 0, st, a, out, w, h, ik, r);
}
void launch_extend_wrap(hipStream_t st, const uchar4* img, const uint8_t* alpha, int cols, int rows, uchar4* ext,
                        int extW) {
  if ((cols & 3) == 0 && (extW & 3) == 0 && (reinterpret_cast<uintptr_t>(img) & 15) == 0 && (reinterpret_cast<uintptr_t>(ext) & 15) == 0 &&
      (reinterpret_cast<uintptr_t>(alpha) & 3) == 0)
    hipLaunchKernelGGL(k_extend_wrap_v4, dim3(cdiv(extW / 4, 256), rows), dim3(256), 0, st, reinterpret_cast<const uint4*>(img),
                       reinterpret_cast<const unsigned*>(alpha), cols / 4, rows, reinterpret_cast<uint4*>(ext), extW / 4);
  else
    hipLaunchKernelGGL(k_extend_wrap, dim3(cdiv(extW, 256), rows), dim3(256), 0, st, img, alpha, cols, rows, ext, extW);
}
void launch_pole_warp_packed(hipStream_t st, const uchar4* extFisheye, const float2* flow, uchar4* warpedExt,
                             const PoleWarpParams& pw, const DevTables& T, unsigned* packed, void* tiles) {
  MapFromPoleFlow mf{flow, pw};
  const int nt = (int)remap_packed_tiles(pw.extW, pw.rows);
  hipLaunchKernelGGL((k_remap_pack<MapFromPoleFlow>), dim3(cdiv(pw.extW, PT_W), cdiv(pw.rows, PT_H), 1), dim3(PT_W, PT_TY), 0, st,
                     mf, pw.extW, pw.rows, pw.extW, pw.rows, packed, reinterpret_cast<int4*>(tiles), (size_t)0, nt);
  hipLaunchKernelGGL((k_remap_cubic_u8c4_packed<MapFromPoleFlow, 0, false>), dim3(cdiv(pw.extW, PT_W), cdiv(pw.rows, PT_H), 1),
                     dim3(PT_W, PT_TY), 0, st, extFisheye, pw.extW, pw.rows, packed, reinterpret_cast<const int4*>(tiles), mf,
                     warpedExt, pw.extW, pw.rows, T.bicubic_i, 0, 1, (size_t)0, (size_t)0, nt, T.bicubic_w1, T.bicubic_res);
}
void launch_pole_finish(hipStream_t st, const uchar4* warpedExt, uchar4* out, int eqrH, const PoleWarpParams& pw) {
  if ((pw.cols & 3) == 0 && (pw.extW & 3) == 0 && pw.cols + ((pw.maxBlendX + 3) & ~3) <= pw.extW &&
      (reinterpret_cast<uintptr_t>(warpedExt) & 15) == 0 && (reinterpret_cast<uintptr_t>(out) & 15) == 0)
    hipLaunchKernelGGL(k_pole_finish_v4, dim3(cdiv(pw.cols / 4, 256), eqrH), dim3(256), 0, st,
                       reinterpret_cast<const uint4*>(warpedExt), reinterpret_cast<uint4*>(out), eqrH, pw);
  else
    hipLaunchKernelGGL(k_pole_finish, dim3(cdiv(pw.cols, 256), eqrH), dim3(256), 0, st, warpedExt, out, eqrH, pw);
}
void launch_flatten(hipStream_t st, const uchar4* base, const uchar4* top, uchar4* out, int w, int h, int flip_top,
                    const DevTables& T) {
  if ((w & 3) == 0)
    hipLaunchKernelGGL(k_flatten_v4, dim3(cdiv(w / 4, 256), h), dim3(256), 0, st, reinterpret_cast<const uint4*>(base),
                       reinterpret_cast<const uint4*>(top), reinterpret_cast<uint4*>(out), w / 4, h, flip_top, T);
  else
    hipLaunchKernelGGL(k_flatten, dim3(cdiv(w, 256), h), dim3(256), 0, st, base, top, out, w, h, flip_top, T);
}
void launch_cubemap(hipStream_t st, const uchar4* eyeL, const uchar4* eyeR, int sw, int sh, const float2* maps, int fw,
                    int fh, int video, uint8_t* out, const DevTables& T) {
  const int ow = video ? 3 * fw : fw, oh = video ? 4 * fh : 12 * fh;
  hipLaunchKernelGGL(k_cubemap, dim3(cdiv(ow, 256), oh), dim3(256), 0, st, eyeL, eyeR, sw, sh, maps, fw, fh, video, out, ow,
                     oh, T.bicubic_i);
}
static CubeGeom cube_geom(int fw, int fh, int video) {
  CubeGeom G;
  G.fw = fw; G.fh = fh; G.video = video;
  G.ow = video ? 3 * fw : fw;
  G.eyeH = video ? 2 * fh : 6 * fh;
  G.txN = (int)cdiv(fw, CT_W);
  G.tyN = (int)cdiv(fh, CT_H);
  return G;
}
size_t cubemap_tile_count(int fw, int fh) { return (size_t)6 * cdiv(fw, CT_W) * cdiv(fh, CT_H); }
int cubemap_lds_pixels() {
  static const int cap = [] {
    const char* e = std::getenv("S360_CUBEMAP_LDS_PIXELS");
    return e && std::atoi(e) == 2560 ? 2560 : 4096;
  }();
  return cap;
}
void launch_cubemap_pack(hipStream_t st, const float2* maps, int sw, int sh, int fw, int fh, int video, int lds_pixels,
                         unsigned* packed, void* tiles) {
  const CubeGeom G = cube_geom(fw, fh, video);
  const dim3 grid(G.txN, G.tyN, 6);
  if (lds_pixels == 2560)
    hipLaunchKernelGGL(k_cubemap_pack<2560>, grid, dim3(64), 0, st, maps, sw, sh, G, packed, static_cast<int4*>(tiles));
  else
    hipLaunchKernelGGL(k_cubemap_pack<4096>, grid, dim3(64), 0, st, maps, sw, sh, G, packed, static_cast<int4*>(tiles));
}
void launch_cubemap_tiles(hipStream_t st, const uchar4* const* eyes, uint8_t* const* outs, int n, int sw, int sh,
                          const float2* maps, const unsigned* packed, const void* tiles, int fw, int fh, int video,
                          int lds_pixels, const DevTables& T) {
  const CubeGeom G = cube_geom(fw, fh, video);
  for (int i = 0; i < n; i += kCubeMaxSlots) {
    const int m = std::min(kCubeMaxSlots, n - i);
    CubeJobs J = {};
    for (int k = 0; k < m; ++k) {
      J.eye[2 * k] = eyes[2 * (i + k)];
      J.eye[2 * k + 1] = eyes[2 * (i + k) + 1];
      J.out[k] = outs[i + k];
    }
    const dim3 grid(G.txN, 6 * G.tyN, 2 * m);
    if (lds_pixels == 2560)
      hipLaunchKernelGGL(k_cubemap_tiles<2560>, grid, dim3(64), 0, st, J, sw, sh, maps, packed, static_cast<const int4*>(tiles), G,
                         T.bicubic_i);
    else
      hipLaunchKernelGGL(k_cubemap_tiles<4096>, grid, dim3(64), 0, st, J, sw, sh, maps, packed, static_cast<const int4*>(tiles), G,
                         T.bicubic_i);
  }
}
void launch_pack_bgr(hipStream_t st, const uchar4* src, int w, int h, uint8_t* dst) {
  const size_t n = (size_t)w * h;
  if ((n & 3) == 0 && (reinterpret_cast<uintptr_t>(dst) & 3) == 0 && (reinterpret_cast<uintptr_t>(src) & 15) == 0)
    hipLaunchKernelGGL(k_pack_bgr_v4, dim3(cdiv(n / 4, 256)), dim3(256), 0, st, reinterpret_cast<const uint4*>(src), n / 4,
                       reinterpret_cast<unsigned*>(dst));
  else
    hipLaunchKernelGGL(k_pack_bgr, dim3(cdiv(n, 256)), dim3(256), 0, st, src, n, dst);
}
int sharpen_max_images() { return IIR_MAX_IMGS; }
size_t sharpen_scratch_bytes(int w, int h) {
  return std::max(iir_waves(h) * iir_tiles(w), iir_waves(w) * iir_tiles(h)) * 64 * sizeof(float);
}
void launch_sharpen_many(hipStream_t st, uchar4* const* imgs, uchar4* const* lps, float* const* scratch, int n, int w,
                         int h, float amount) {
  if (n < 1 || n > IIR_MAX_IMGS) throw std::runtime_error("launch_sharpen_many: 1..32 images per launch");
  const float alpha = powf(0.25f, 1.0f / 4.0f);
  const IirGeom gr{w, h, w}, gc{h, w, w};
  IirImgs rows, cols;
  for (int i = 0; i < IIR_MAX_IMGS; ++i) {
    const int k = i < n ? i : 0;
    rows.x[i] = imgs[k]; rows.out[i] = lps[k]; rows.ck[i] = scratch[k];
    cols.x[i] = lps[k]; cols.out[i] = imgs[k]; cols.ck[i] = scratch[k];
  }
  hipLaunchKernelGGL((k_iir_pass<true, false>), dim3(cdiv(h, IIR_CH), n), dim3(64), 0, st, rows, gr, alpha, amount);
  hipLaunchKernelGGL((k_iir_pass<false, true>), dim3(cdiv(w, IIR_CH), n), dim3(64), 0, st, cols, gc, alpha, amount);
}
void launch_sharpen(hipStream_t st, uchar4* img, uchar4* lp, float* scratch, int w, int h, float amount) {
  launch_sharpen_many(st, &img, &lp, &scratch, 1, w, h, amount);
}

}
```

surround360_amd/csrc/render_kernels.hpp:

```cpp
#pragma once
#include <hip/hip_runtime.h>
#include <stddef.h>
#include <stdint.h>

namespace s360 {

struct DevCamera {
  int type;
  double pos[3], R[9], principal[2], focal[2], distortion[2];
};
struct DevTables {
  const short* bicubic_i;
  const float* bicubic_w1;
  const short* bicubic_res;
  const float* bicubic_f;
  const float* tanh10;
  const float* tanh5;
  const float* flat_softmaxL;
};
struct NovelViewParams {
  int overlapW, camH, stripW, numNovelViews;
  int numPairs;
  int numLocal;
  float camImageWidthHalf;
  float disp;
};
struct PoleWarpParams {
  int cols, rows, extW, maxBlendX;
  float poleCameraRadius, phiRampStart, phiMid, phiRampEnd;
};

void launch_bgr_to_bgra(hipStream_t st, const uint8_t* src, int channels, uchar4* dst, size_t n);
void launch_u16_high_byte(hipStream_t st, const unsigned short* src, uint8_t* dst, size_t n);
void launch_prepare_side_src(hipStream_t st, const uint8_t* src, int channels, uchar4* dst, int w, int h, int feather);
void launch_spherical_map(hipStream_t st, float2* map, int dw, int dh, const DevCamera& cam, const float* cosX,
                          const float* sinX, const float* cosY, const float* sinY);
void launch_remap_cubic_u8c4(hipStream_t st, const uchar4* src, int sw, int sh, const float2* map, uchar4* dst, int dw,
                             int dh, const DevTables& T, int alpha_mode, int yFeatherStart, int featherSize,
                             int batch = 1 );
size_t remap_packed_tiles(int dw, int dh);
void launch_remap_pack_map(hipStream_t st, const float2* map, int sw, int sh, int dw, int dh, unsigned* packed, void* tiles,
                           int batch = 1);
void launch_remap_cubic_u8c4_packed(hipStream_t st, const uchar4* src, int sw, int sh, const float2* map, const unsigned* packed,
                                    const void* tiles, uchar4* dst, int dw, int dh, const DevTables& T, int alpha_mode,
                                    int yFeatherStart, int featherSize, int batch = 1);
void launch_crop_overlaps(hipStream_t st, const uchar4* proj, int camW, int camH, int P, int overlapW, uchar4* out,
                          int p0, int p1);
void launch_novel_view(hipStream_t st, const uchar4* overlaps, const float2* flows ,
                       uchar4* strips, const NovelViewParams& nv, int p0, int p1, const DevTables& T);
void launch_morph_views(hipStream_t st, const uchar4* imgL, const uchar4* imgR, const float2* flowLtoR, const float2* flowRtoL,
                        int w, int h, const double* shifts, int n, uchar4* merged, uchar4* fromL, uchar4* fromR,
                        const DevTables& T, int views_per_block = 0);
void launch_assemble_pano(hipStream_t st, const uchar4* strips_eye, int P, int camH, int stripW, float offset,
                          uchar4* pano, int eqrW, int eqrH);
void launch_flip_both(hipStream_t st, const uchar4* src, uchar4* dst, int w, int h, int rows);
void launch_erode_alpha(hipStream_t st, const uchar4* img, uint8_t* out, int w, int h, int e);
void launch_gauss_u8(hipStream_t st, const uint8_t* a, uint8_t* out, int w, int h, const int* ik, int r);
void launch_extend_wrap(hipStream_t st, const uchar4* img, const uint8_t* alpha , int cols, int rows,
                        uchar4* ext, int extW);
void launch_pole_warp_packed(hipStream_t st, const uchar4* extFisheye, const float2* flow, uchar4* warpedExt,
                             const PoleWarpParams& pw, const DevTables& T, unsigned* packed ,
                             void* tiles );
void launch_pole_finish(hipStream_t st, const uchar4* warpedExt, uchar4* out, int eqrH, const PoleWarpParams& pw);
void launch_flatten(hipStream_t st, const uchar4* base, const uchar4* top, uchar4* out, int w, int h, int flip_top,
                    const DevTables& T);
void launch_cubemap(hipStream_t st, const uchar4* eyeL, const uchar4* eyeR, int sw, int sh, const float2* maps, int fw,
                    int fh, int video, uint8_t* out, const DevTables& T);
constexpr int kCubeMaxSlots = 16;
size_t cubemap_tile_count(int fw, int fh);
int cubemap_lds_pixels();
void launch_cubemap_pack(hipStream_t st, const float2* maps, int sw, int sh, int fw, int fh, int video, int lds_pixels,
                         unsigned* packed, void* tiles);
void launch_cubemap_tiles(hipStream_t st, const uchar4* const* eyes, uint8_t* const* outs, int n, int sw, int sh,
                          const float2* maps, const unsigned* packed, const void* tiles, int fw, int fh, int video,
                          int lds_pixels, const DevTables& T);
void launch_remap_by_flow(hipStream_t st, const uchar4* src, int w, int h, const float2* flow, uchar4* dst,
                          const DevTables& T);
void launch_red_mask(hipStream_t st, const uint8_t* bgr, uint8_t* red, size_t n);
void launch_circle_alpha(hipStream_t st, const uchar4* src, const uint8_t* red , uchar4* dst, int w, int h,
                         float radius);
void launch_pole_removal_combine(hipStream_t st, uchar4* bottom, const uchar4* warped2, size_t n);
void launch_pack_bgr(hipStream_t st, const uchar4* src, int w, int h, uint8_t* dst);
int sharpen_max_images();
size_t sharpen_scratch_bytes(int w, int h);
void launch_sharpen_many(hipStream_t st, uchar4* const* imgs, uchar4* const* lps, float* const* scratch, int n, int w,
                         int h, float amount);
void launch_sharpen(hipStream_t st, uchar4* img, uchar4* lp, float* scratch, int w, int h, float amount);

}
```

Baseline: 52.50.

## Remap pole spheres directly into extended buffer and skip padding rows

Top/bottom spherical remaps now write straight into the extended-image slots with a pitched destination, and a small wrap-strip kernel fills only the wrap columns. This replaces the intermediate topSph/botSph buffers and the full extend-wrap copy. Pole finish now writes the zero padding rows only when the buffer is new or the row count changed. Flatten skips reading top-layer rows beyond the valid pole rows. Debug readers get pitched copies instead. The cost is more bookkeeping and a reliance on the padding rows staying zero across frames.

```diff
diff --git a/surround360_amd/csrc/api.hip b/surround360_amd/csrc/api.hip
--- a/surround360_amd/csrc/api.hip
+++ b/surround360_amd/csrc/api.hip
@@ -604,7 +604,7 @@
     c->op_a.ensure(n * 4); c->op_b.ensure(n * 4); c->op_c.ensure(n * 4);
     h2d(c, c->op_a.p, bottom_layer, n * 4);
     h2d(c, c->op_b.p, top_layer, n * 4);
-    launch_flatten(c->st, c->op_a.as<uchar4>(), c->op_b.as<uchar4>(), c->op_c.as<uchar4>(), w, h, 0, F.tab.dev);
+    launch_flatten(c->st, c->op_a.as<uchar4>(), c->op_b.as<uchar4>(), c->op_c.as<uchar4>(), w, h, 0, h, F.tab.dev);
     d2h(c, out, c->op_c.p, n * 4);
   });
 }
@@ -1206,11 +1206,12 @@
     d2h(c, out_bgr, frame_state(c).cubeOut.p, (size_t)ow * oh * 3);
   });
 }
-static const void* frame_u8_source(s360_ctx* c, FrameState& F, const std::string& n, int idx, bool pack_eye, int& w, int& h, int& ch) {
+static const void* frame_u8_source(s360_ctx* c, FrameState& F, const std::string& n, int idx, bool pack_eye, int& w, int& h, int& ch,
+                                   int& pitch) {
   const s360_geometry& g = c->g;
   const int W = c->P.eqr_width, H = c->P.eqr_height, P = F.P;
   const void* src = nullptr;
-  w = 0; h = 0; ch = 4;
+  w = 0; h = 0; ch = 4; pitch = 0;
   const int nloc = F.side_p1 - F.side_p0;
   if (n == "projection") {
     need(idx >= 0 && idx < P && F.sc->proj.p, "projection not available");
@@ -1226,9 +1227,11 @@
     need(F.panoDbg[e].p, "enable keep_intermediates before rendering");
     w = W; h = H; src = F.panoDbg[e].p;
   } else if (n == "top_spherical") {
-    need(F.sc->topSph.p, "not available"); w = W; h = g.top_rows; src = F.sc->topSph.p;
+    need(F.haveTopSph && F.extImgs[F.last_pole].p, "not available"); w = W; h = g.top_rows; pitch = F.extW;
+    src = F.extImgs[F.last_pole].as<uchar4>() + F.extStride * 4;
   } else if (n == "bottom_spherical") {
-    need(F.sc->botSph.p, "not available"); w = W; h = g.bottom_rows; src = F.sc->botSph.p;
+    need(F.haveBotSph && F.extImgs[F.last_pole].p, "not available"); w = W; h = g.bottom_rows; pitch = F.extW;
+    src = F.extImgs[F.last_pole].as<uchar4>() + F.extStride * 5;
   } else if (n == "pole_warped") {
     need(idx >= 0 && idx < 4 && F.sc->poleWarped[idx].p, "not available"); w = W; h = H; src = F.sc->poleWarped[idx].p;
   } else if (n == "extended_side" || n == "extended_fisheye") {
@@ -1253,15 +1256,23 @@
   } else {
     throw Error(S360_ERR_INVALID_ARG, "unknown intermediate name: " + n);
   }
+  if (!pitch) pitch = w;
   return src;
 }
 int s360_frame_get_u8(s360_ctx* c, const char* name, int idx, int whc[3], uint8_t* dst) {
   return frame_guard(c, [&] {
     need(c && name && whc, "bad argument");
-    int w = 0, h = 0, ch = 4;
-    const void* src = frame_u8_source(c, frame_state(c), name, idx, dst != nullptr, w, h, ch);
+    int w = 0, h = 0, ch = 4, pitch = 0;
+    const void* src = frame_u8_source(c, frame_state(c), name, idx, dst != nullptr, w, h, ch, pitch);
     whc[0] = w; whc[1] = h; whc[2] = ch;
-    if (dst) d2h(c, dst, src, (size_t)w * h * ch);
+    if (dst && pitch != w) {
+      wait_finish_stream(c);
+      S360_HIP(hipMemcpy2DAsync(dst, (size_t)w * ch, src, (size_t)pitch * ch, (size_t)w * ch, (size_t)h, hipMemcpyDeviceToHost, c->st));
+      S360_HIP(hipStreamSynchronize(c->st));
+      check_sweep_error(c);
+    } else if (dst) {
+      d2h(c, dst, src, (size_t)w * h * ch);
+    }
   });
 }
 size_t s360_png_bound_c(int w, int h, int channels) {
@@ -1390,19 +1401,34 @@
     FrameState& F = frame_state(c);
     std::vector<PngPlan> plans;
     std::vector<const uint8_t*> px;
+    std::vector<int> pitches;
     for (int i = 0; i < n; ++i) {
       need(names[i] != nullptr, "bad argument");
-      int w = 0, h = 0, ch = 0;
-      const void* src = frame_u8_source(c, F, names[i], idx[i], false, w, h, ch);
+      int w = 0, h = 0, ch = 0, pitch = 0;
+      const void* src = frame_u8_source(c, F, names[i], idx[i], false, w, h, ch, pitch);
       need(ch == 4 && src, "only the 4-channel intermediates are encoded as state images");
       plans.push_back(PngPlan::make(w, h, 4));
       px.push_back(static_cast<const uint8_t*>(src));
+      pitches.push_back(pitch == w ? 0 : pitch);
     }
     s360_ctx::PngBatch& B = c->statePng;
     png_batch_prepare(c, B, plans);
     if (c->st2) {
       S360_HIP(hipEventRecord(B.evAfter, c->st2));
       S360_HIP(hipStreamWaitEvent(c->st, B.evAfter, 0));
+    }
+    size_t packBytes = 0, packAt = 0;
+    for (int i = 0; i < n; ++i)
+      if (pitches[(size_t)i]) packBytes += ((size_t)plans[(size_t)i].w * plans[(size_t)i].h * 4 + 15) & ~(size_t)15;
+    if (packBytes) F.sc->sphPacked.ensure(packBytes);
+    for (int i = 0; i < n; ++i) {
+      if (!pitches[(size_t)i]) continue;
+      const size_t rowBytes = (size_t)plans[(size_t)i].w * 4;
+      uint8_t* d = F.sc->sphPacked.as<uint8_t>() + packAt;
+      S360_HIP(hipMemcpy2DAsync(d, rowBytes, px[(size_t)i], (size_t)pitches[(size_t)i] * 4, rowBytes, (size_t)plans[(size_t)i].h,
+                                hipMemcpyDeviceToDevice, c->st));
+      px[(size_t)i] = d;
+      packAt += (rowBytes * plans[(size_t)i].h + 15) & ~(size_t)15;
     }
     png_batch_run(c, B, px.data());
   });
diff --git a/surround360_amd/csrc/render.hip b/surround360_amd/csrc/render.hip
--- a/surround360_amd/csrc/render.hip
+++ b/surround360_amd/csrc/render.hip
@@ -617,7 +617,7 @@
 }
 
 void dev_pole_unit_post(s360_ctx* c, const uchar4* extFisheye, const float2* flow, int cols, int rows, int extW,
-                        uchar4* warped_out, int eqrH) {
+                        uchar4* warped_out, int eqrH, bool write_padding) {
   FrameState& F = frame_state(c);
   PoleWarpParams pw;
   pw.cols = cols; pw.rows = rows; pw.extW = extW;
@@ -631,7 +631,7 @@
   F.sc->warpTiles.ensure(remap_packed_tiles(extW, rows) * 16);
   launch_pole_warp_packed(c->st, extFisheye, flow, F.sc->warpedExt.as<uchar4>(), pw, F.tab.dev, F.sc->warpPacked.as<unsigned>(),
                           F.sc->warpTiles.p);
-  launch_pole_finish(c->st, F.sc->warpedExt.as<uchar4>(), warped_out, eqrH, pw);
+  launch_pole_finish(c->st, F.sc->warpedExt.as<uchar4>(), warped_out, eqrH, pw, write_padding);
 }
 
 namespace {
@@ -704,6 +704,7 @@
       }
     if (!pole_mask) continue;
     const int cur = F.cur_pole;
+    F.haveTopSph = F.haveBotSph = false;
     F.extImgs[cur].ensure(6 * xs * sizeof(uchar4));
     F.poleFlows.ensure(4 * xs * sizeof(float2));
     uchar4* ext = F.extImgs[cur].as<uchar4>();
@@ -712,31 +713,31 @@
       ProfScope ps(prof, "project_pole");
       if (pole_mask & 3) {
         if (!F.have_top) throw Error(S360_ERR_STATE, "top image not uploaded");
-        F.sc->topSph.ensure((size_t)W * rowsT * sizeof(uchar4));
         const int yfs = rowsT - 1 - c->P.std_alpha_feather_size;
         s360_ctx::PackedMap& pk = ensure_packed(c, c->topPk, c->topMap.as<float2>(), F.topW, F.topH, W, rowsT, 1, st);
         launch_remap_cubic_u8c4_packed(st, F.topSrc.as<uchar4>(), F.topW, F.topH, c->topMap.as<float2>(),
-                                       pk.packed.as<unsigned>(), pk.tiles.p, F.sc->topSph.as<uchar4>(), W, rowsT,
-                                       F.tab.dev, 1, yfs, c->P.std_alpha_feather_size);
-        launch_extend_wrap(st, F.sc->topSph.as<uchar4>(), nullptr, W, rowsT, ext + 4 * xs, extW);
+                                       pk.packed.as<unsigned>(), pk.tiles.p, ext + 4 * xs, W, rowsT,
+                                       F.tab.dev, 1, yfs, c->P.std_alpha_feather_size, 1, extW);
+        launch_wrap_strip(st, ext + 4 * xs, W, rowsT, extW);
+        F.haveTopSph = true;
       }
       if (pole_mask & 12) {
         if (!F.have_bottom) throw Error(S360_ERR_STATE, "bottom image not uploaded");
-        F.sc->botSph.ensure((size_t)W * rowsB * sizeof(uchar4));
         const int yfs = rowsB - 1 - c->P.std_alpha_feather_size;
         if (c->P.enable_pole_removal) {
           dev_pole_removal(c, F, use_prev != 0);
           s360_ctx::PackedMap& pk = ensure_packed(c, c->botPk, c->botMap.as<float2>(), F.poleW, F.poleH, W, rowsB, 1, st);
           launch_remap_cubic_u8c4_packed(st, F.prMerged.as<uchar4>(), F.poleW, F.poleH, c->botMap.as<float2>(),
-                                         pk.packed.as<unsigned>(), pk.tiles.p, F.sc->botSph.as<uchar4>(), W, rowsB,
-                                         F.tab.dev, 2, yfs, c->P.std_alpha_feather_size);
+                                         pk.packed.as<unsigned>(), pk.tiles.p, ext + 5 * xs, W, rowsB,
+                                         F.tab.dev, 2, yfs, c->P.std_alpha_feather_size, 1, extW);
         } else {
           s360_ctx::PackedMap& pk = ensure_packed(c, c->botPk, c->botMap.as<float2>(), F.poleW, F.poleH, W, rowsB, 1, st);
           launch_remap_cubic_u8c4_packed(st, F.botSrc.as<uchar4>(), F.poleW, F.poleH, c->botMap.as<float2>(),
-                                         pk.packed.as<unsigned>(), pk.tiles.p, F.sc->botSph.as<uchar4>(), W, rowsB,
-                                         F.tab.dev, 1, yfs, c->P.std_alpha_feather_size);
+                                         pk.packed.as<unsigned>(), pk.tiles.p, ext + 5 * xs, W, rowsB,
+                                         F.tab.dev, 1, yfs, c->P.std_alpha_feather_size, 1, extW);
         }
-        launch_extend_wrap(st, F.sc->botSph.as<uchar4>(), nullptr, W, rowsB, ext + 5 * xs, extW);
+        launch_wrap_strip(st, ext + 5 * xs, W, rowsB, extW);
+        F.haveBotSph = true;
       }
     }
     {
@@ -813,9 +814,12 @@
         ProfScope ps(prof, "pole_warp");
         for (int u = 0; u < 4; ++u)
           if (pole_mask & (1 << u)) {
+            const void* had = F.sc->poleWarped[u].p;
             F.sc->poleWarped[u].ensure(en * sizeof(uchar4));
+            const bool pad = F.sc->poleWarped[u].p != had || F.sc->polePadRows[u] != rowsOf(u);
             dev_pole_unit_post(c, ext + (u < 2 ? 4 : 5) * xs, F.poleFlows.as<float2>() + u * xs, W, rowsOf(u), extW,
-                               F.sc->poleWarped[u].as<uchar4>(), H);
+                               F.sc->poleWarped[u].as<uchar4>(), H, pad);
+            F.sc->polePadRows[u] = rowsOf(u);
             F.poleFrame[u] = F.frames_done;
             F.sc->poleOwner[u] = &F;
           }
@@ -838,13 +842,13 @@
       for (int e = 0; e < 2; ++e) {
         if (composite_mask & (1 << e)) {
           launch_flatten(st, F.pano[e].as<uchar4>(), F.sc->poleWarped[e].as<uchar4>(), F.sc->panoTmp.as<uchar4>(), W, H, 0,
-                         F.tab.dev);
+                         rowsT, F.tab.dev);
           std::swap(F.pano[e].p, F.sc->panoTmp.p);
           std::swap(F.pano[e].cap, F.sc->panoTmp.cap);
         }
         if (composite_mask & (4 << e)) {
           launch_flatten(st, F.pano[e].as<uchar4>(), F.sc->poleWarped[2 + e].as<uchar4>(), F.sc->panoTmp.as<uchar4>(), W, H, 1,
-                         F.tab.dev);
+                         rowsB, F.tab.dev);
           std::swap(F.pano[e].p, F.sc->panoTmp.p);
           std::swap(F.pano[e].cap, F.sc->panoTmp.cap);
         }
diff --git a/surround360_amd/csrc/render.hpp b/surround360_amd/csrc/render.hpp
--- a/surround360_amd/csrc/render.hpp
+++ b/surround360_amd/csrc/render.hpp
@@ -23,8 +23,9 @@
 struct SlotScratch {
   DevBuf proj;
   DevBuf panoFlip[2], panoTmp;
-  DevBuf topSph, botSph;
+  DevBuf sphPacked;
   DevBuf warpedExt, poleWarped[4];
+  int polePadRows[4] = {-1, -1, -1, -1};
   const void* poleOwner[4] = {nullptr, nullptr, nullptr, nullptr};
   DevBuf warpPacked, warpTiles;
   DevBuf eyeFinal[2];
@@ -73,6 +74,7 @@
   bool keep_intermediates = false;
   DevBuf panoDbg[2];
   int extW = 0, poleRowsT = 0, poleRowsB = 0;
+  bool haveTopSph = false, haveBotSph = false;
   size_t extStride = 0;
   DevBuf botSrc2, prRed[2], prImgs[2], prFlow[2], prTmp, prWarp, prMerged;
   bool have_pr_inputs = false, have_prev_pr = false;
@@ -117,7 +119,7 @@
                               int erode_size = -1, const int* taps = nullptr);
 std::vector<int> feather_gauss_taps(int erode_size);
 void dev_pole_unit_post(s360_ctx* c, const uchar4* extFisheye, const float2* flow, int cols, int rows, int extW,
-                        uchar4* warped_out , int eqrH);
+                        uchar4* warped_out , int eqrH, bool write_padding = true);
 
 bool host_is_pinned(const void* p, size_t bytes);
 
diff --git a/surround360_amd/csrc/render_kernels.hip b/surround360_amd/csrc/render_kernels.hip
--- a/surround360_amd/csrc/render_kernels.hip
+++ b/surround360_amd/csrc/render_kernels.hip
@@ -365,12 +365,13 @@
                                                                          const short* __restrict__ tab,
                                                                          int yFeatherStart, int featherSize, size_t sbs,
                                                                          size_t dbs, int tilesPerImage,
-                                                                         const float* __restrict__ w1, const short* __restrict__ wres) {
+                                                                         const float* __restrict__ w1, const short* __restrict__ wres,
+                                                                         int dpitch) {
   __shared__ __attribute__((aligned(16))) float s_w1[WT ? 256 : 4];
   __shared__ short s_res[WT ? 1024 : 2];
   const TileId tile = xcd_tile();
   src += sbs * tile.z;
-  dst += dbs * tile.z;
+  dst += (size_t)dpitch * dh * tile.z;
   packed += dbs * tile.z;
   mapfn.advance(dbs * tile.z);
   __shared__ uchar4 s_tile[PT_CAP];
@@ -491,7 +492,7 @@
         o.w = o.w < a ? o.w : a;
       }
     }
-    dst[(size_t)y * dw + x] = o;
+    dst[(size_t)y * dpitch + x] = o;
   }
 }
 
@@ -1111,6 +1112,16 @@
   if (alpha) p.w = alpha[(size_t)y * cols + sx];
   ext[(size_t)y * extW + x] = p;
 }
+__global__ __launch_bounds__(256) void k_wrap_strip(uchar4* __restrict__ ext, int cols, int extW) {
+  const int x = cols + blockIdx.x * blockDim.x + threadIdx.x, y = blockIdx.y;
+  if (x >= extW) return;
+  ext[(size_t)y * extW + x] = ext[(size_t)y * extW + x % cols];
+}
+__global__ __launch_bounds__(256) void k_wrap_strip_v4(uint4* __restrict__ ext, int cols4, int extW4) {
+  const int x = cols4 + blockIdx.x * blockDim.x + threadIdx.x, y = blockIdx.y;
+  if (x >= extW4) return;
+  ext[(size_t)y * extW4 + x] = ext[(size_t)y * extW4 + x % cols4];
+}
 
 __global__ __launch_bounds__(256) void k_extend_wrap_v4(const uint4* __restrict__ img, const unsigned* __restrict__ alpha,
                                                         int cols4, int rows, uint4* __restrict__ ext, int extW4) {
@@ -1188,24 +1199,31 @@
   return o;
 }
 __global__ __launch_bounds__(256) void k_flatten(const uchar4* __restrict__ base, const uchar4* __restrict__ top,
-                                                 uchar4* __restrict__ out, int w, int h, int flip_top, DevTables T) {
+                                                 uchar4* __restrict__ out, int w, int h, int flip_top, int top_rows,
+                                                 DevTables T) {
   const int x = blockIdx.x * blockDim.x + threadIdx.x, y = blockIdx.y;
   if (x >= w) return;
   const uchar4 b = base[(size_t)y * w + x];
-  const uchar4 t = flip_top ? top[(size_t)(h - 1 - y) * w + (w - 1 - x)] : top[(size_t)y * w + x];
+  const int ty = flip_top ? h - 1 - y : y;
+  uchar4 t = make_uchar4(0, 0, 0, 0);
+  if (ty < top_rows) t = flip_top ? top[(size_t)ty * w + (w - 1 - x)] : top[(size_t)ty * w + x];
   out[(size_t)y * w + x] = flatten_px(b, t, T);
 }
 __global__ __launch_bounds__(256) void k_flatten_v4(const uint4* __restrict__ base, const uint4* __restrict__ top,
-                                                    uint4* __restrict__ out, int w4, int h, int flip_top, DevTables T) {
+                                                    uint4* __restrict__ out, int w4, int h, int flip_top, int top_rows,
+                                                    DevTables T) {
   const int x4 = blockIdx.x * blockDim.x + threadIdx.x, y = blockIdx.y;
   if (x4 >= w4) return;
   const uint4 b = base[(size_t)y * w4 + x4];
-  uint4 t;
-  if (flip_top) {
-    const uint4 r = top[(size_t)(h - 1 - y) * w4 + (w4 - 1 - x4)];
-    t = make_uint4(r.w, r.z, r.y, r.x);
-  } else {
-    t = top[(size_t)y * w4 + x4];
+  const int ty = flip_top ? h - 1 - y : y;
+  uint4 t = make_uint4(0u, 0u, 0u, 0u);
+  if (ty < top_rows) {
+    if (flip_top) {
+      const uint4 r = top[(size_t)ty * w4 + (w4 - 1 - x4)];
+      t = make_uint4(r.w, r.z, r.y, r.x);
+    } else {
+      t = top[(size_t)ty * w4 + x4];
+    }
   }
   uint4 o;
   o.x = __builtin_bit_cast(unsigned, flatten_px(__builtin_bit_cast(uchar4, b.x), __builtin_bit_cast(uchar4, t.x), T));
@@ -1656,8 +1674,9 @@
 }
 void launch_remap_cubic_u8c4_packed(hipStream_t st, const uchar4* src, int sw, int sh, const float2* map, const unsigned* packed,
                                     const void* tiles, uchar4* dst, int dw, int dh, const DevTables& T, int alpha_mode,
-                                    int yFeatherStart, int featherSize, int batch) {
+                                    int yFeatherStart, int featherSize, int batch, int dst_pitch) {
   MapFromBuffer mf{map, dw};
+  const int dpitch = dst_pitch > 0 ? dst_pitch : dw;
   const dim3 grid(cdiv(dw, PT_W), cdiv(dh, PT_H), batch), block(PT_W, PT_TY);
   const int4* t4 = reinterpret_cast<const int4*>(tiles);
   const size_t sbs = (size_t)sw * sh, dbs = (size_t)dw * dh;
@@ -1665,7 +1684,7 @@
   const bool wt = remap_rebuild_weights() && T.bicubic_res;
 #define S360_RP(A, W)                                                                                                              \
   hipLaunchKernelGGL((k_remap_cubic_u8c4_packed<MapFromBuffer, A, W>), grid, block, 0, st, src, sw, sh, packed, t4, mf, dst, dw, dh, \
-                     T.bicubic_i, yFeatherStart, featherSize, sbs, dbs, nt, T.bicubic_w1, T.bicubic_res)
+                     T.bicubic_i, yFeatherStart, featherSize, sbs, dbs, nt, T.bicubic_w1, T.bicubic_res, dpitch)
   if (alpha_mode == 1) { if (wt) S360_RP(1, true); else S360_RP(1, false); }
   else if (alpha_mode == 2) { if (wt) S360_RP(2, true); else S360_RP(2, false); }
   else { if (wt) S360_RP(0, true); else S360_RP(0, false); }
@@ -1744,6 +1763,14 @@
   else
     hipLaunchKernelGGL(k_extend_wrap, dim3(cdiv(extW, 256), rows), dim3(256), 0, st, img, alpha, cols, rows, ext, extW);
 }
+void launch_wrap_strip(hipStream_t st, uchar4* ext, int cols, int rows, int extW) {
+  if (extW <= cols) return;
+  if ((cols & 3) == 0 && (extW & 3) == 0 && (reinterpret_cast<uintptr_t>(ext) & 15) == 0)
+    hipLaunchKernelGGL(k_wrap_strip_v4, dim3(cdiv((extW - cols) / 4, 256), rows), dim3(256), 0, st, reinterpret_cast<uint4*>(ext),
+                       cols / 4, extW / 4);
+  else
+    hipLaunchKernelGGL(k_wrap_strip, dim3(cdiv(extW - cols, 256), rows), dim3(256), 0, st, ext, cols, extW);
+}
 void launch_pole_warp_packed(hipStream_t st, const uchar4* extFisheye, const float2* flow, uchar4* warpedExt,
                              const PoleWarpParams& pw, const DevTables& T, unsigned* packed, void* tiles) {
   MapFromPoleFlow mf{flow, pw};
@@ -1752,23 +1779,25 @@
                      mf, pw.extW, pw.rows, pw.extW, pw.rows, packed, reinterpret_cast<int4*>(tiles), (size_t)0, nt);
   hipLaunchKernelGGL((k_remap_cubic_u8c4_packed<MapFromPoleFlow, 0, false>), dim3(cdiv(pw.extW, PT_W), cdiv(pw.rows, PT_H), 1),
                      dim3(PT_W, PT_TY), 0, st, extFisheye, pw.extW, pw.rows, packed, reinterpret_cast<const int4*>(tiles), mf,
-                     warpedExt, pw.extW, pw.rows, T.bicubic_i, 0, 1, (size_t)0, (size_t)0, nt, T.bicubic_w1, T.bicubic_res);
-}
-void launch_pole_finish(hipStream_t st, const uchar4* warpedExt, uchar4* out, int eqrH, const PoleWarpParams& pw) {
+                     warpedExt, pw.extW, pw.rows, T.bicubic_i, 0, 1, (size_t)0, (size_t)0, nt, T.bicubic_w1, T.bicubic_res, pw.extW);
+}
+void launch_pole_finish(hipStream_t st, const uchar4* warpedExt, uchar4* out, int eqrH, const PoleWarpParams& pw,
+                        bool write_padding) {
+  const int outRows = write_padding ? eqrH : min(pw.rows, eqrH);
   if ((pw.cols & 3) == 0 && (pw.extW & 3) == 0 && pw.cols + ((pw.maxBlendX + 3) & ~3) <= pw.extW &&
       (reinterpret_cast<uintptr_t>(warpedExt) & 15) == 0 && (reinterpret_cast<uintptr_t>(out) & 15) == 0)
-    hipLaunchKernelGGL(k_pole_finish_v4, dim3(cdiv(pw.cols / 4, 256), eqrH), dim3(256), 0, st,
+    hipLaunchKernelGGL(k_pole_finish_v4, dim3(cdiv(pw.cols / 4, 256), outRows), dim3(256), 0, st,
                        reinterpret_cast<const uint4*>(warpedExt), reinterpret_cast<uint4*>(out), eqrH, pw);
   else
-    hipLaunchKernelGGL(k_pole_finish, dim3(cdiv(pw.cols, 256), eqrH), dim3(256), 0, st, warpedExt, out, eqrH, pw);
+    hipLaunchKernelGGL(k_pole_finish, dim3(cdiv(pw.cols, 256), outRows), dim3(256), 0, st, warpedExt, out, eqrH, pw);
 }
 void launch_flatten(hipStream_t st, const uchar4* base, const uchar4* top, uchar4* out, int w, int h, int flip_top,
-                    const DevTables& T) {
+                    int top_rows, const DevTables& T) {
   if ((w & 3) == 0)
     hipLaunchKernelGGL(k_flatten_v4, dim3(cdiv(w / 4, 256), h), dim3(256), 0, st, reinterpret_cast<const uint4*>(base),
-                       reinterpret_cast<const uint4*>(top), reinterpret_cast<uint4*>(out), w / 4, h, flip_top, T);
+                       reinterpret_cast<const uint4*>(top), reinterpret_cast<uint4*>(out), w / 4, h, flip_top, top_rows, T);
   else
-    hipLaunchKernelGGL(k_flatten, dim3(cdiv(w, 256), h), dim3(256), 0, st, base, top, out, w, h, flip_top, T);
+    hipLaunchKernelGGL(k_flatten, dim3(cdiv(w, 256), h), dim3(256), 0, st, base, top, out, w, h, flip_top, top_rows, T);
 }
 void launch_cubemap(hipStream_t st, const uchar4* eyeL, const uchar4* eyeR, int sw, int sh, const float2* maps, int fw,
                     int fh, int video, uint8_t* out, const DevTables& T) {
diff --git a/surround360_amd/csrc/render_kernels.hpp b/surround360_amd/csrc/render_kernels.hpp
--- a/surround360_amd/csrc/render_kernels.hpp
+++ b/surround360_amd/csrc/render_kernels.hpp
@@ -43,7 +43,7 @@
                            int batch = 1);
 void launch_remap_cubic_u8c4_packed(hipStream_t st, const uchar4* src, int sw, int sh, const float2* map, const unsigned* packed,
                                     const void* tiles, uchar4* dst, int dw, int dh, const DevTables& T, int alpha_mode,
-                                    int yFeatherStart, int featherSize, int batch = 1);
+                                    int yFeatherStart, int featherSize, int batch = 1, int dst_pitch = 0);
 void launch_crop_overlaps(hipStream_t st, const uchar4* proj, int camW, int camH, int P, int overlapW, uchar4* out,
                           int p0, int p1);
 void launch_novel_view(hipStream_t st, const uchar4* overlaps, const float2* flows ,
@@ -58,12 +58,14 @@
 void launch_gauss_u8(hipStream_t st, const uint8_t* a, uint8_t* out, int w, int h, const int* ik, int r);
 void launch_extend_wrap(hipStream_t st, const uchar4* img, const uint8_t* alpha , int cols, int rows,
                         uchar4* ext, int extW);
+void launch_wrap_strip(hipStream_t st, uchar4* ext, int cols, int rows, int extW);
 void launch_pole_warp_packed(hipStream_t st, const uchar4* extFisheye, const float2* flow, uchar4* warpedExt,
                              const PoleWarpParams& pw, const DevTables& T, unsigned* packed ,
                              void* tiles );
-void launch_pole_finish(hipStream_t st, const uchar4* warpedExt, uchar4* out, int eqrH, const PoleWarpParams& pw);
+void launch_pole_finish(hipStream_t st, const uchar4* warpedExt, uchar4* out, int eqrH, const PoleWarpParams& pw,
+                        bool write_padding = true);
 void launch_flatten(hipStream_t st, const uchar4* base, const uchar4* top, uchar4* out, int w, int h, int flip_top,
-                    const DevTables& T);
+                    int top_rows, const DevTables& T);
 void launch_cubemap(hipStream_t st, const uchar4* eyeL, const uchar4* eyeR, int sw, int sh, const float2* maps, int fw,
                     int fh, int video, uint8_t* out, const DevTables& T);
 constexpr int kCubeMaxSlots = 16;
```

Result: no change. 52.87, median of 6 (+0.7%).
